# mattsaccount364/FractalShark

Measured on AMD Instinct MI355X. Metric: Mpix/s (iteration buffer), View #5 3840x2160 HDRx32 LAv2, higher is better.
Workload: dtype f32+i32exp; 1 GPU; view5_3840x2160_hdrx32_lav2_full; parity=cpu, kernel_variant=tuned, frames=warm: frames of one view back to back

## Files before the change

fractalshark_amd/_capi.py:

```python
import ctypes as C
import os

from . import _build

vp = C.c_void_p
u32 = C.c_uint32
u64 = C.c_uint64
i32 = C.c_int32


class RealHdr32(C.Structure):
    _fields_ = [("m", C.c_float), ("e", C.c_int32)]


class CplxHdr32(C.Structure):
    _fields_ = [("re", C.c_float), ("im", C.c_float), ("e", C.c_int32)]


class AtHdr32(C.Structure):
    _fields_ = [("StepLength", u32), ("ThresholdC", RealHdr32), ("SqrEscapeRadius", RealHdr32),
                ("RefC", CplxHdr32), ("ZCoeff", CplxHdr32), ("CCoeff", CplxHdr32), ("InvZCoeff", CplxHdr32),
                ("CCoeffSqrInvZCoeff", CplxHdr32), ("CCoeffInvZCoeff", CplxHdr32),
                ("CCoeffNormSqr", RealHdr32), ("RefCNormSqr", RealHdr32), ("factor", RealHdr32)]

# ... 55 lines not shown
    fn.argtypes = argtypes
    return fn


def render_lib():
    global _render
    if _render is not None:
        return _render
    path = os.environ.get("FSMI355_LIB") or _build.LIB_RENDER
    if os.environ.get("FSMI355_LIB"):
        import sys
        print("fractalshark_amd: FSMI355_LIB overrides the in-tree library: %s" % path, file=sys.stderr)
    if not os.path.exists(path):
        raise RuntimeError("libfsmi355.so is missing (%s): run `python -c 'import __graft_entry__ as g; g.build()'`"
                           % path)
    lib = C.CDLL(path)
    _decl(lib, "fs_create", vp, [C.c_int])
    _decl(lib, "fs_destroy", None, [vp])
    _decl(lib, "fs_test_device_is_working", u32, [])
    _decl(lib, "fs_device_count", C.c_int, [])
    _decl(lib, "fs_host_fallback_bytes", u64, [vp])
    _decl(lib, "fs_idle_device_bytes", u64, [vp])
    _decl(lib, "fs_release_idle_device_memory", u64, [C.c_int])
    _decl(lib, "fs_set_compressed_orbit_mode", u32, [vp, C.c_int])
    _decl(lib, "fs_orbit_device_bytes", u64, [vp])
    _decl(lib, "fs_error_string", C.c_char_p, [u32])
    _decl(lib, "fs_init_memory", u32, [vp, u32, u32, u32, u32, vp, u32, u32, u64, C.c_int])
    _decl(lib, "fs_set_row_bands", u32, [vp, u32, u32, u32])
    _decl(lib, "fs_local_rows", u32, [vp])
    _decl(lib, "fs_set_external_iter_buffer", u32, [vp, vp, u64])
    _decl(lib, "fs_device_iter_buffer", vp, [vp])
    _decl(lib, "fs_rounded_width", u32, [vp])
    _decl(lib, "fs_upload_orbit", u32, [vp, u64, C.c_int, u32, vp, u64, u64, u64])
    _decl(lib, "fs_upload_orbit_compressed", u32, [vp, u64, C.c_int, u32, vp, u64, u64, u64, vp, vp])
    _decl(lib, "fs_upload_la", u32, [vp, u64, C.c_int, u32, vp, u32, vp, u32, C.c_int, C.c_int, vp])
    _decl(lib, "fs_upload_bla", u32, [vp, C.c_int, vp, vp, i32, i32])
    _decl(lib, "fs_render_lav2", u32, [vp, C.c_int, C.c_int, C.c_int, vp, u64])
    _decl(lib, "fs_feature_eval", u32, [vp, C.c_int, u32, C.c_int, vp, u64, vp, vp, u64])
    _decl(lib, "fs_feature_eval_direct", u32, [vp, C.c_int, u32, C.c_int, vp, u64, vp, vp, u64])
    _decl(lib, "fs_set_feature_slice", u32, [vp, u32])
    _decl(lib, "fs_autozoom_pick", u32, [vp, C.c_int, u64, vp, C.POINTER(AutozoomResult)])
    _decl(lib, "fs_set_autozoom_gather_cap", u32, [vp, u32])
    _decl(lib, "fs_render_exact", u32, [vp, u32, u32, u32, vp, vp, u32, C.c_int, u64])
    _decl(lib, "fs_exact_stable_mask", u32, [vp, u32, u32, vp, vp, u32, u64, vp])
    _decl(lib, "fs_set_exact_slice", u32, [vp, u32, C.c_int])
    _decl(lib, "fs_read_exact_stats", u32, [vp, vp])
    _decl(lib, "fs_exact_sample_counts", u32, [vp, u32, u32, vp, vp, u32, u32, C.c_int, u64, vp])
    _decl(lib, "fs_render_exact_wide", u32, [vp, u32, u32, u32, vp, vp, u32, C.c_int, u64])
    _decl(lib, "fs_exact_wide_state", u32, [vp, u32, u32, vp, vp, u32, u32, vp, vp])
    _decl(lib, "fs_render_bla", u32, [vp, C.c_int, vp, u64])
    _decl(lib, "fs_render_direct", u32, [vp, C.c_int, vp, u64])
    _decl(lib, "fs_upload_orbit_scaled", u32, [vp, C.c_int, u32, vp, vp, u64, u64])
    _decl(lib, "fs_render_scaled", u32, [vp, C.c_int, vp, u64])
    _decl(lib, "fs_build_bla", u32, [vp, C.c_int, vp])
    _decl(lib, "fs_bla_num_levels", i32, [vp])
    _decl(lib, "fs_bla_lm2", i32, [vp])
    _decl(lib, "fs_bla_level_size", u64, [vp, i32])
    _decl(lib, "fs_read_bla_level", u32, [vp, i32, vp, u64])
    _decl(lib, "fs_render_direct_lp", u32, [vp, C.c_int, vp, u64, C.c_int])
    _decl(lib, "fs_clear", u32, [vp])
    _decl(lib, "fs_render_current", u32, [vp, u64, vp, vp, vp, C.c_int])
    _decl(lib, "fs_sync_compute", u32, [vp])
    _decl(lib, "fs_compute_stream", vp, [vp])
    _decl(lib, "fs_sync_display", u32, [vp])
    _decl(lib, "fs_query_compute", u32, [vp])
    _decl(lib, "fs_enqueue_done_callback", u32, [vp, DONE_CB, vp])
    _decl(lib, "fs_get_width", u32, [vp])
    _decl(lib, "fs_get_height", u32, [vp])
    _decl(lib, "fs_last_kernel_ms", C.c_float, [vp])
    _decl(lib, "fs_set_kernel_variant", u32, [vp, C.c_int])
    _decl(lib, "fs_kernel_ms_history", u32, [vp, vp, u32])
    _decl(lib, "fs_kernel_ms_split_history", u32, [vp, vp, vp, u32])
    _decl(lib, "fs_forget_tile_costs", u32, [vp])
    _decl(lib, "fs_last_frame_tile_ordered", C.c_int, [vp])
    _decl(lib, "fs_last_frame_sampled_tile_order", C.c_int, [vp])
    _decl(lib, "fs_read_tile_costs", u32, [vp, vp, u64, vp])
    _decl(lib, "fs_read_tile_order", u32, [vp, vp, u64])
    _decl(lib, "fs_seq_cursor_probe", u32, [vp, C.c_int, u64, u32, vp])
    _decl(lib, "fs_enable_step_count", u32, [vp, C.c_int])
    _decl(lib, "fs_read_step_count", u32, [vp, vp])
    _decl(lib, "fs_time_render_current", u32, [vp, u64, u32, vp])
    _decl(lib, "fs_read_stats_raw", u32, [vp, vp, u64])
    _decl(lib, "fs_test_block_threshold", u32, [vp, vp, vp, vp, vp, u32])
    _decl(lib, "fs_build_la", u32, [vp, C.c_int, vp, C.c_int])
    _decl(lib, "fs_build_la_mt", u32, [vp, C.c_int, vp, C.c_int, C.c_int])
    _decl(lib, "fs_la_counts", u32, [vp, vp, vp, vp, vp])
    _decl(lib, "fs_read_la", u32, [vp, vp, u32, vp, u32, vp])
    _decl(lib, "fs_group_create", vp, [vp, C.c_int, C.c_int])
    _decl(lib, "fs_group_destroy", None, [vp])
    _decl(lib, "fs_group_size", C.c_int, [vp])
    _decl(lib, "fs_group_transport", C.c_int, [vp])
    _decl(lib, "fs_group_renderer", vp, [vp, C.c_int])
    _decl(lib, "fs_group_init_memory", u32, [vp, u32, u32, u32, u32, vp, u32, u32, u64])
    _decl(lib, "fs_group_upload_orbit", u32, [vp, u64, C.c_int, u32, vp, u64, u64, u64])
    _decl(lib, "fs_group_upload_orbit_compressed", u32, [vp, u64, C.c_int, u32, vp, u64, u64, u64, vp, vp])
    _decl(lib, "fs_group_upload_la", u32, [vp, u64, C.c_int, u32, vp, u32, vp, u32, C.c_int, C.c_int, vp])
    _decl(lib, "fs_group_upload_bla", u32, [vp, C.c_int, vp, vp, i32, i32])
    _decl(lib, "fs_group_upload_orbit_scaled", u32, [vp, C.c_int, u32, vp, vp, u64, u64])
    _decl(lib, "fs_group_render_lav2", u32, [vp, C.c_int, C.c_int, C.c_int, vp, u64])
    _decl(lib, "fs_group_render_bla", u32, [vp, C.c_int, vp, u64])
    _decl(lib, "fs_group_render_scaled", u32, [vp, C.c_int, vp, u64])
    _decl(lib, "fs_group_render_direct", u32, [vp, C.c_int, vp, u64])
    _decl(lib, "fs_group_clear", u32, [vp])
    _decl(lib, "fs_group_render_current", u32, [vp, u64, vp, vp])
    _decl(lib, "fs_group_render_current_colors", u32, [vp, u64, vp, vp, vp, C.c_int])
    _decl(lib, "fs_group_sync_display", u32, [vp])
    _decl(lib, "fs_display_stream", vp, [vp])
    _decl(lib, "fs_colorize_frame", u32, [vp, vp, u64, vp, vp, vp])
    _decl(lib, "fs_color_buffer_elements", u64, [vp])
    _decl(lib, "fs_group_sync", u32, [vp])
    _decl(lib, "fs_group_wait_current", u32, [vp, u32])
    _decl(lib, "fs_group_gather_ms", C.c_float, [vp])
    _decl(lib, "fs_group_plan", None, [u32, u32, u32, u32, vp, vp, vp])
    _decl(lib, "fs_group_set_host_path", u32, [vp, C.c_int])
    _decl(lib, "fs_group_host_path", C.c_int, [vp])
    _decl(lib, "fs_copy_bands_to_host", u32, [vp, vp, vp, vp])
    _decl(lib, "fs_host_register", u32, [vp, u64])
    _decl(lib, "fs_host_unregister", u32, [vp])
    _render = lib
    return lib


RENDER_SYMBOLS = [
    "fs_create", "fs_destroy", "fs_test_device_is_working", "fs_device_count", "fs_error_string", "fs_init_memory", "fs_set_row_bands",
    "fs_local_rows", "fs_set_external_iter_buffer", "fs_device_iter_buffer", "fs_rounded_width", "fs_upload_orbit", "fs_upload_orbit_compressed",
    "fs_upload_la", "fs_upload_bla", "fs_render_lav2", "fs_feature_eval", "fs_feature_eval_direct", "fs_set_feature_slice",
    "fs_autozoom_pick", "fs_set_autozoom_gather_cap",
    "fs_render_exact", "fs_exact_stable_mask", "fs_set_exact_slice", "fs_read_exact_stats",
    "fs_exact_sample_counts", "fs_render_exact_wide", "fs_exact_wide_state",
    "fs_render_bla", "fs_render_direct", "fs_upload_orbit_scaled",
    "fs_render_scaled", "fs_build_bla", "fs_bla_num_levels", "fs_bla_lm2", "fs_bla_level_size", "fs_read_bla_level",
    "fs_render_direct_lp", "fs_clear",
    "fs_render_current", "fs_sync_compute", "fs_compute_stream", "fs_sync_display", "fs_query_compute", "fs_enqueue_done_callback",
    "fs_host_fallback_bytes", "fs_idle_device_bytes", "fs_release_idle_device_memory", "fs_set_compressed_orbit_mode", "fs_orbit_device_bytes", "fs_get_width", "fs_get_height", "fs_last_kernel_ms", "fs_set_kernel_variant", "fs_kernel_ms_history", "fs_kernel_ms_split_history", "fs_forget_tile_costs", "fs_last_frame_tile_ordered", "fs_last_frame_sampled_tile_order", "fs_read_tile_costs", "fs_read_tile_order", "fs_seq_cursor_probe", "fs_enable_step_count", "fs_read_step_count",
    "fs_time_render_current", "fs_read_stats_raw", "fs_test_block_threshold", "fs_build_la", "fs_build_la_mt", "fs_la_counts", "fs_read_la",
    "fs_group_create", "fs_group_destroy", "fs_group_size", "fs_group_transport", "fs_group_renderer", "fs_group_init_memory",
    "fs_group_upload_orbit", "fs_group_upload_orbit_compressed", "fs_group_upload_la", "fs_group_upload_bla",
    "fs_group_upload_orbit_scaled", "fs_group_render_lav2", "fs_group_render_bla", "fs_group_render_scaled",
    "fs_group_render_direct", "fs_group_clear", "fs_group_render_current", "fs_group_render_current_colors", "fs_group_sync_display", "fs_display_stream", "fs_colorize_frame",
    "fs_color_buffer_elements", "fs_group_sync", "fs_group_wait_current", "fs_group_gather_ms",
    "fs_group_plan", "fs_group_set_host_path", "fs_group_host_path", "fs_copy_bands_to_host", "fs_host_register", "fs_host_unregister",
]


def inputs_lib():
    global _inputs
    if _inputs is not None:
        return _inputs
    path = _build.LIB_INPUTS
    if not os.path.exists(path):
        raise RuntimeError("libfsinputs.so is missing (%s): run __graft_entry__.build()" % path)
    lib = C.CDLL(path)
    _decl(lib, "fsh_view_create", vp, [C.c_char_p] * 4 + [u32, u32])
    _decl(lib, "fsh_view_destroy", None, [vp])
    _decl(lib, "fsh_view_autozoom_next", vp, [vp, C.c_double, C.c_double, u32, u32, u32])
    _decl(lib, "fsh_view_save_im", C.c_int, [vp, u64, C.c_char_p, C.c_int])
    _decl(lib, "fsh_view_load_im", vp, [C.c_char_p, u32, u32, C.POINTER(u64), C.POINTER(C.c_int), C.POINTER(C.c_int)])
    _decl(lib, "fsh_view_precision_bits", u64, [vp])
    _decl(lib, "fsh_view_exact_axes", C.c_int, [vp, u32, u32, u32, C.c_int, u32, vp, vp])
    _decl(lib, "fsh_view_bbox_str", C.c_int, [vp, C.c_int, C.c_char_p, C.c_size_t])
    _decl(lib, "fsh_view_coords_direct_f64", None, [vp, u32, u32, vp])
    _decl(lib, "fsh_view_coords_direct_hdr32", None, [vp, u32, u32, vp])
    _decl(lib, "fsh_view_coords_direct_hdr64", None, [vp, u32, u32, vp])
    _decl(lib, "fsh_orbit_create", vp, [vp, C.c_int, u64, C.c_int])
    _decl(lib, "fsh_orbit_create_ex", vp, [vp, C.c_int, u64, C.c_int, C.c_int])
    _decl(lib, "fsh_orbit_is_compressed", C.c_int, [vp])
    _decl(lib, "fsh_orbit_compressed_count", u64, [vp])
    _decl(lib, "fsh_orbit_compressed_data_hdr32", vp, [vp])
    _decl(lib, "fsh_orbit_low_hdr32", None, [vp, vp])
    _decl(lib, "fsh_orbit_compressed_data_hdr64", vp, [vp])
    _decl(lib, "fsh_orbit_low_hdr64", None, [vp, vp])
    _decl(lib, "fsh_la_default_params", None, [C.POINTER(C.c_int32)])
    _decl(lib, "fsh_mpz_raw_write", C.c_size_t, [C.c_char_p, C.c_int, C.c_char_p, C.c_size_t])
    _decl(lib, "fsh_mpz_raw_read", C.c_size_t, [C.c_char_p, C.c_size_t, C.c_char_p, C.c_size_t])
    _decl(lib, "fsh_orbit_save_im", C.c_int, [vp, u64, C.c_int, C.c_char_p, C.c_int])
    _decl(lib, "fsh_orbit_load_im", vp, [C.c_char_p, C.POINTER(u64)])
    _decl(lib, "fsh_orbit_is64", C.c_int, [vp])
    _decl(lib, "fsh_orbit_destroy", None, [vp])
    _decl(lib, "fsh_feature_begin", vp, [vp, vp, u32, u32, u32, u64])
    _decl(lib, "fsh_feature_begin_direct", vp, [vp, C.c_int, u32, u32, u32, u64])
    _decl(lib, "fsh_feature_begin_direct_at", vp, [vp, C.c_int, u32, u32, u32, u64])
    _decl(lib, "fsh_feature_direct_grid", C.c_int, [vp, C.c_int, u32, u32, vp, vp])
    _decl(lib, "fsh_feature_destroy", None, [vp])
    _decl(lib, "fsh_feature_is64", C.c_int, [vp])
    _decl(lib, "fsh_feature_candidates", u64, [vp])
    _decl(lib, "fsh_feature_next_batch", u64, [vp, vp, u64, C.POINTER(C.c_int), vp, C.POINTER(u64)])
    _decl(lib, "fsh_feature_consume", None, [vp, vp, u64])
    _decl(lib, "fsh_feature_found", u64, [vp])
    _decl(lib, "fsh_feature_result", C.c_int, [vp, u64, C.c_char_p, C.c_char_p, C.c_char_p, C.c_size_t, C.POINTER(u64),
                                                vp, C.POINTER(u32)])
    _decl(lib, "fsh_orbit_count", u64, [vp])
    _decl(lib, "fsh_orbit_scale_entries", u64, [vp, vp, vp, u64])
    _decl(lib, "fsh_orbit_period", u64, [vp])
    _decl(lib, "fsh_orbit_data_hdr32", vp, [vp])
    _decl(lib, "fsh_orbit_data_hdr64", vp, [vp])
    _decl(lib, "fsh_orbit_max_radius_hdr32", None, [vp, vp])
    _decl(lib, "fsh_orbit_max_radius_hdr64", None, [vp, vp])
    _decl(lib, "fsh_orbit_data_hdr32_bad", vp, [vp])
    _decl(lib, "fsh_orbit_data_f32_bad", vp, [vp])
    _decl(lib, "fsh_orbit_bad_count", u64, [vp])
    _decl(lib, "fsh_view_coords_direct_lp", None, [vp, u32, u32, C.c_int, vp])
    _decl(lib, "fsh_view_coords_perturb_hdr32", None, [vp, vp, u32, u32, vp])
    _decl(lib, "fsh_view_coords_perturb_hdr64", None, [vp, vp, u32, u32, vp])
    _decl(lib, "fsh_df32_op", None, [C.c_int, vp, vp, vp])
    _decl(lib, "fsh_hr2_reduce", None, [vp])
    _decl(lib, "fsh_hr2_add", None, [vp, vp, C.c_int, vp])
    _decl(lib, "fsh_hc2_reduce", None, [vp])
    _decl(lib, "fsh_convert_orbit_hdr64_to_2x32", None, [vp, u64, vp])
    _decl(lib, "fsh_convert_la_hdr64_to_2x32", None, [vp, u64, vp])
    _decl(lib, "fsh_convert_at_hdr64_to_2x32", None, [vp, vp])
    _decl(lib, "fsh_view_coords_perturb_2x32", None, [vp, vp, u32, u32, vp])
    _decl(lib, "fsh_la_create_hdr32", vp, [vp, C.c_int])
    _decl(lib, "fsh_la_create", vp, [vp, C.c_int])
    _decl(lib, "fsh_la_create_ex", vp, [vp, C.c_int, C.c_int])
    _decl(lib, "fsh_la_is64", C.c_int, [vp])
    _decl(lib, "fsh_la_destroy", None, [vp])
    _decl(lib, "fsh_la_count", u32, [vp])
    _decl(lib, "fsh_la_data", vp, [vp])
# ... 55 lines not shown
```

fractalshark_amd/csrc/kernels.h:

```cpp
#pragma once

#include <hip/hip_runtime.h>
#include <stdint.h>

#include "../../include/fs_layout.h"
#include "exact_math.hpp"
#include "exact_wide_math.hpp"
#include "hdr_math.hpp"

enum { FS_MODE_FULL = 0, FS_MODE_PO = 1, FS_MODE_LAO = 2 };
enum { FS_PARITY_LITERAL = 0, FS_PARITY_GPUSTAGE = 1 };
enum { FS_VARIANT_TUNED = 0, FS_VARIANT_LITERAL = 1, FS_VARIANT_TUNED_NOSCALE = 2, FS_VARIANT_BASE_MASK = 0xff };
enum { FS_VARIANT_FLAG_LDS_ORBIT = 0x100, FS_VARIANT_FLAG_REFILL = 0x200, FS_VARIANT_FLAG_WIDE = 0x400,
       FS_VARIANT_FLAG_NATURAL_ORDER = 0x800, FS_VARIANT_FLAG_BLA_POOL = 0x1000 };

struct FsFrame {
    uint32_t width;
    uint32_t height;
    uint32_t rounded_width;
    uint32_t local_rows;
    uint32_t band_first;
    uint32_t band_rows;
    uint32_t band_stride;
    uint32_t iter_u64;
    uint32_t wide;
};

struct FsZ64 {
    double re;
    double im;
    int32_t e;
    int32_t pad_;
    double w;
};
template <class F> struct FsDev;
template <> struct FsDev<float> {
    using Z = float4;
    using Orbit = fs_orbit_hdr32;
    using Real = fs_real_hdr32;
    using Cplx = fs_cplx_hdr32;
    using LA = fs_la_hdr32_u32;
    using AT = fs_at_hdr32_u32;
    using BLA = fs_bla_hdr32;
};
template <> struct FsDev<double> {
    using Z = FsZ64;
    using Orbit = fs_orbit_hdr64;
    using Real = fs_real_hdr64;
    using Cplx = fs_cplx_hdr64;
    using LA = fs_la_hdr64_u32;
    using AT = fs_at_hdr64_u32;
    using BLA = fs_bla_hdr64;
};

template <class F> struct FsFeatRec;
template <> struct FsFeatRec<float> {
    using In = fs_feature_in_hdr32;
    using Out = fs_feature_out_hdr32;
};
template <> struct FsFeatRec<double> {
    using In = fs_feature_in_hdr64;
    using Out = fs_feature_out_hdr64;
};
template <class F> struct FsFeatLane {
    fs::hcplx<F> z, dz, dzdc, zcoeff, dc, c;
    fs::hreal<F> sqr_r, sqr_scale;
    uint64_t step, cap, period;
    uint32_t ref, phase;
};
template <class F> struct FsFeatDirectLane {
    fs::hcplx<F> z, dzdc, zcoeff, c;
    uint64_t step, cap, period;
    uint32_t phase, pad_;
};

template <class F> struct FsCoordsT {
    fs::hreal<F> dx, dy, centerX, centerY;
};
using FsCoords32 = FsCoordsT<float>;

struct FsAtRes {
    double re, im;
    int32_t e;
    uint32_t i;
};
template <class F> struct FsLav2ArgsT {
    uint32_t *out;
    const typename FsDev<F>::Z *zref;
    const float4 *zq;
    const float4 *zs;
    const float2 *zs2;
    const float4 *zqb;
    const typename FsDev<F>::LA *las;
    const fs_la_stage_u32 *stages;
    uint64_t *stats;
    FsFrame frame;
    FsCoordsT<F> coords;
    typename FsDev<F>::AT at;
    uint32_t orbit_count;
    uint32_t period;
    uint32_t stage_count;
    uint32_t n_iterations;
    uint32_t n_iterations_hi;
    int la_valid;
    int use_at;
    int parity;
    const void *wp;
    uint32_t n_wp;
    typename FsDev<F>::Real cxLow, cyLow;
    const uint32_t *tile_order;
    uint32_t *tile_cost;
    uint32_t tiles_x;
    const uint32_t *pixel_order;
    uint32_t *pixel_cost;
    struct FsAtRes *at_res;
    uint32_t *at_cost;
    uint32_t orbit_count_hi, period_hi, at_step_hi, la_u64;
};
using FsLav2Args32 = FsLav2ArgsT<float>;
template <class F> struct FsLaU64;
template <> struct FsLaU64<float> {
    using T = fs_la_hdr32_u64;
};
template <> struct FsLaU64<double> {
    using T = fs_la_hdr64_u64;
};

struct FsBlaRec {
    float Axm, Aym, Bxm, Bym;
    int32_t Axe, Aye, Bxe, Bye;
    float Zre, Zim;
    int32_t Ze;
    uint32_t l;
};
static_assert(sizeof(FsBlaRec) == 48, "device-native BLA record");
constexpr int kBlaMaxLevels = 40;

template <class F> struct FsBlaArgsT {
    uint32_t *out;
    const typename FsDev<F>::Z *zref;
    const float4 *zq;
    const float4 *zs;
    const float2 *zs2;
    const float4 *zqb;
    const typename FsDev<F>::BLA *const *levels;
    uint64_t *stats;
    uint32_t *queue;
    const uint32_t *tile_order;
    uint32_t *probe_out;
    uint32_t probe_pitch;
    FsFrame frame;
    FsCoordsT<F> coords;
    uint32_t orbit_count;
    uint32_t n_iterations;
    uint32_t n_iterations_hi;
    int32_t lm2;
    const FsBlaRec *nrec;
    const int4 *nlad;
    const long long *nkmax;
    uint32_t level_off[kBlaMaxLevels];
    const float4 *zb;
    const int4 *hq;
    const int4 *hlad;
    const FsBlaRec *hrec;
};
using FsBlaArgs32 = FsBlaArgsT<float>;

struct FsBlaArgsF64 {
    uint32_t *out;
    const fs_orbit_f64 *orbit;
    const fs_bla_f64 *const *levels;
    uint64_t *stats;
    FsFrame frame;
    double dx, dy, centerX, centerY;
    uint32_t orbit_count;
    uint32_t n_iterations;
    uint32_t n_iterations_hi;
    int32_t lm2;
};

template <class F> struct FsDirectHdrArgsT {
    uint32_t *out;
    fs::hreal<F> *cx_row;
    uint64_t *stats;
    FsFrame frame;
    fs::hreal<F> dy;
    fs::hreal<F> maxY;
    uint32_t n_iterations;
    uint32_t n_iterations_hi;
};

struct FsLav2Args2x32 {
    uint32_t *out;
    const fs_orbit_2x32 *orbit;
    const fs_la_2x32_u32 *las;
    const fs_la_stage_u32 *stages;
    uint64_t *stats;
    FsFrame frame;
    fs_real_2x32 coords[4];
    fs_at_2x32_u32 at;
    uint32_t orbit_count;
    uint32_t stage_count;
    uint32_t n_iterations;
    uint32_t n_iterations_hi;
    int la_valid;
    int use_at;
    const fs_orbit_2x32_rc *wp;
    uint32_t n_wp;
    fs_real_2x32 cxLow, cyLow;
    const uint32_t *pixel_order;
    uint32_t *pixel_cost;
    const uint32_t *tile_order;
    uint32_t tiles_x;
};

struct FsLav2ArgsPlain {
    uint32_t *out;
    const void *orbit;
    const void *las;
    const fs_la_stage_u32 *stages;
    uint64_t *stats;
    FsFrame frame;
    alignas(8) uint8_t at[sizeof(fs_at_f64_u32)];
    alignas(8) uint8_t coords[4 * sizeof(double)];
    uint32_t orbit_count;
    uint32_t stage_count;
    uint32_t n_iterations;
    uint32_t n_iterations_hi;
    int la_valid;
    int use_at;
    const void *wp;
    uint32_t n_wp;
    alignas(8) uint8_t c_low[2][8];
};

struct FsScaledArgs32 {
    uint32_t *out;
    const fs_orbit_hdr32_bad *orbit_t;
    const fs_orbit_f32_bad *orbit_f;
    uint64_t *stats;
    FsFrame frame;
    FsCoordsT<float> coords;
    uint32_t orbit_count;
    uint32_t n_iterations;
    uint32_t n_iterations_hi;
    float w2threshold;
};

struct FsScaledArgsF64 {
    uint32_t *out;
    const fs_orbit_f64_bad *orbit_t;
    const fs_orbit_f32_bad *orbit_f;
    uint64_t *stats;
    FsFrame frame;
    double dx, dy, centerX, centerY;
    uint32_t orbit_count;
    uint32_t n_iterations;
    uint32_t n_iterations_hi;
    float w2threshold;
};

struct FsDirectLpArgs {
    uint32_t *out;
    uint64_t *stats;
    FsFrame frame;
    float c32[16];
    double c64[16];
    uint32_t n_iterations;
    uint32_t n_iterations_hi;
};

struct FsDirectArgs64 {
    uint32_t *out;
    double *cx_row;
    uint64_t *stats;
    FsFrame frame;
    double dy;
    double maxY;
    uint32_t n_iterations;
    uint32_t n_iterations_hi;
};

void fsk_prepare_orbit_hdr32(const fs_orbit_hdr32 *in, float4 *out, uint64_t n, hipStream_t s);
void fsk_decompress_orbit_plain(int type_tag, const void *wp, uint64_t n_wp, uint64_t n_uncompressed, const void *cxLow,
                                const void *cyLow, void *out, hipStream_t s);
void fsk_decompress_orbit_hdr32(const fs_orbit_hdr32_rc *wp, uint64_t n_wp, uint64_t n_uncompressed, fs_real_hdr32 cxLow,
                                fs_real_hdr32 cyLow, float4 *out, hipStream_t s);
void fsk_decompress_orbit_hdr64(const fs_orbit_hdr64_rc *wp, uint64_t n_wp, uint64_t n_uncompressed, fs_real_hdr64 cxLow,
                                fs_real_hdr64 cyLow, FsZ64 *out, hipStream_t s);
void fsk_prepare_orbit_hdr64(const fs_orbit_hdr64 *in, FsZ64 *out, uint64_t n, hipStream_t s);
template <class F>
void fsk_feature_init(const void *in, FsFeatLane<F> *st, void *out, uint64_t n, int find, fs::hreal<F> R, uint64_t max_iters,
                      uint64_t count, hipStream_t s);
template <class F>
void fsk_feature_step(const typename FsDev<F>::Z *zref, uint32_t count, FsFeatLane<F> *st, void *out, uint64_t n, int find,
                      int iter_u64, uint32_t slice, uint32_t *unfinished, hipStream_t s);
template <class F>
void fsk_feature_direct_init(const void *in, FsFeatDirectLane<F> *st, void *out, uint64_t n, int find, fs::hreal<F> R,
                             uint64_t max_iters, hipStream_t s);
template <class F>
void fsk_feature_direct_step(FsFeatDirectLane<F> *st, void *out, uint64_t n, int find, int iter_u64, fs::hreal<F> R,
                             uint32_t slice, uint32_t *unfinished, hipStream_t s);
void fsk_make_quiet_orbit(const float4 *zref, float4 *zq, float2 *zs2, float4 *zqb, uint64_t n, hipStream_t s);
void fsk_tile_order(const uint32_t *probe, uint32_t probe_pitch, uint32_t tiles_x, uint32_t tiles_y, uint32_t threshold,
                    uint32_t *order, uint32_t n_slots, hipStream_t s);
uint32_t fsk_tile_order_work_words(uint32_t n_tiles);
void fsk_tile_order_by_cost(const uint32_t *cost, uint32_t n_tiles, uint32_t *tmp, uint32_t *order, uint32_t n_slots,
                            hipStream_t s);
uint32_t fsk_lav2_hdr32_slots(const FsFrame &f);
void fsk_lav2_hdr32(const FsLav2Args32 &A, int mode, bool stats, int variant, hipStream_t s);
void fsk_lav2_hdr64(const FsLav2ArgsT<double> &A, int mode, bool stats, hipStream_t s);
void fsk_at_pass64(const FsLav2ArgsT<double> &A, hipStream_t s);
void fsk_lav2_wide(const FsLav2Args32 *A32, const FsLav2ArgsT<double> *A64, int mode, bool stats, hipStream_t s);
void fsk_lav2_seq(const FsLav2Args32 *A32, const FsLav2ArgsT<double> *A64, int mode, bool stats, hipStream_t s);
void fsk_seq_cursor_probe(bool is64, bool wide_pos, const void *wp, uint32_t n_wp, const void *cx, const void *cy,
                          uint64_t start, uint32_t n, void *out, hipStream_t s);
void fsk_lav2_2x32(const FsLav2Args2x32 &A, int mode, bool stats, hipStream_t s);
void fsk_lav2_plain(const FsLav2ArgsPlain &A, int kind, int mode, bool stats, hipStream_t s);
bool fsk_direct_lp(const FsDirectLpArgs &A, int kind, int iteration_precision, bool stats, hipStream_t s);
void fsk_scaled_hdr32(const FsScaledArgs32 &A, bool stats, int variant, hipStream_t s);
void fsk_scaled_bounds(fs_orbit_f32_bad *of, uint64_t n, hipStream_t s);
void fsk_scaled_f64(const FsScaledArgsF64 &A, bool stats, int variant, hipStream_t s);
void fsk_bla_build_hdr32(const float4 *zref, void *const *levels, const uint64_t *epl, int n_levels, fs_real_hdr32 bla_size,
                         hipStream_t s);
void fsk_bla_build_hdr64(const FsZ64 *zref, void *const *levels, const uint64_t *epl, int n_levels, fs_real_hdr64 bla_size,
                         hipStream_t s);
void fsk_bla_make_native(const fs_bla_hdr32 *const *levels, const uint32_t *level_off, const uint64_t *epl, int n_levels,
                         const float4 *zref, uint32_t orbit_count, FsBlaRec *rec, int4 *lad, uint32_t *bad, int32_t lm2, long long *kmax, uint32_t n_kmax, hipStream_t s);
void fsk_perturb_scalar_hdr32(const FsBlaArgs32 &A, bool use_bla, bool stats, int variant, hipStream_t s);
uint64_t fsk_bla_heap_positions(const uint64_t *epl, int n_levels);
void fsk_bla_make_heap(const FsBlaRec *rec, const int4 *lad, const long long *kmax, uint32_t n_kmax, const uint32_t *level_off,
                       const uint64_t *epl, int n_levels, int32_t lm2, const float4 *zref, uint32_t orbit_count, FsBlaRec *hrec,
                       int4 *hlad, int4 *hq, float4 *zb, hipStream_t s);
void fsk_bla_hdr32_fast(const FsBlaArgs32 &A, bool pool, hipStream_t s);
struct FsTileSampleArgs {
    FsFrame frame;
    FsCoordsT<double> coords;
    fs::hreal<double> ThresholdC, SqrEscapeRadius;
    fs::hcplx<double> RefC, CCoeff;
    uint32_t StepLength;
    uint32_t n_iterations;
    uint32_t tiles_x, tiles_y;
    uint32_t n_slots;
    uint32_t *cost;
};
void fsk_at_tile_sample64(const FsTileSampleArgs &A, hipStream_t s);
void fsk_tile_order_finish(uint32_t *order, uint32_t n_slots, uint32_t n_tiles, hipStream_t s);
size_t fsk_pixel_order_temp_bytes(uint32_t n);
hipError_t fsk_pixel_order_build(const uint32_t *counts, uint32_t n, uint32_t *work, uint32_t *order, void *temp, size_t temp_bytes,
                                 hipStream_t s);
void fsk_lav2_lit32(const FsLav2Args32 &A, int mode, bool stats, dim3 g, dim3 b, hipStream_t s);
void fsk_lav2_hdr64_fast(const FsLav2ArgsT<double> &A, int mode, bool stats, hipStream_t s);
void fsk_perturb_scalar_hdr64(const FsBlaArgsT<double> &A, bool use_bla, bool stats, int variant, hipStream_t s);
void fsk_perturb_bla_f64(const FsBlaArgsF64 &A, bool use_bla, bool stats, hipStream_t s);
void fsk_direct_hdr32(const FsDirectHdrArgsT<float> &A, fs::hreal<float> minX, fs::hreal<float> dx, bool stats, hipStream_t s);
void fsk_direct_hdr64(const FsDirectHdrArgsT<double> &A, fs::hreal<double> minX, fs::hreal<double> dx, bool stats,
                      hipStream_t s);
void fsk_direct_f64(const FsDirectArgs64 &A, double minX, double dx, bool stats, hipStream_t s);
void fsk_antialias(const void *iters, int iter_u64, uint32_t rounded_width, fs_color16 *colors, const fs_color16 *pal,
                   uint32_t pal_iters, uint32_t aux_depth, uint32_t aa, uint32_t color_w, uint32_t color_h,
                   uint64_t n_iterations, hipStream_t s);
void fsk_reduce(const void *iters, int iter_u64, uint32_t rounded_width, uint32_t width, uint32_t rows,
                fs_reduction *out, hipStream_t s);
struct FsAzStats {
    uint64_t max_iter, sum, n_ge;
    uint64_t num_at_limit, first_index, num_at_max;
    uint64_t candidates, accepted, run_reject, hist[9];
    uint64_t best_key;
    uint64_t gathered;
    double sums[3];
};
struct FsAzTipRec {
    uint32_t x, y;
    uint64_t iter;
    uint32_t high, pad_;
};
struct FsAzFrame {
    const void *iters;
    uint32_t iter_u64, pitch, W, H;
    uint64_t n_iterations;
};
void fsk_az_stats(const FsAzFrame &F, uint32_t x0, uint32_t y0, uint32_t w, uint32_t h, FsAzStats *st, hipStream_t s);
void fsk_az_max(const FsAzFrame &F, FsAzStats *st, hipStream_t s);
void fsk_az_default(const FsAzFrame &F, uint32_t x0, uint32_t y0, uint32_t w, uint32_t h, double width_over_2,
                    double height_over_2, double max_distance, FsAzStats *st, double *slab, hipStream_t s);
void fsk_az_tip_score(const FsAzFrame &F, double max_dist, FsAzStats *st, hipStream_t s);
// ... 3 lines not shown
struct FsExactArgs {
    const uint32_t *cx, *cy;
    uint32_t W, H, rounded_width;
    uint32_t iter_u64;
    void *iters;
    uint64_t cap;
    fsx::Params P;
    const uint32_t *src_xy;
    const uint64_t *src_n;
    const uint32_t *src_pix;
    uint32_t *dst_xy;
    uint64_t *dst_n;
    uint32_t *dst_pix;
    uint32_t stride;
    uint32_t n_src;
    uint32_t first;
    uint32_t compact;
    uint32_t slice;
    uint32_t *dst_count;
    unsigned long long *stats;
};
bool fsk_exact_slice(const FsExactArgs &A, uint32_t limbs, hipStream_t s);
void fsk_exact_mask(const void *centre, const void *shifted, int iter_u64, uint8_t *mask, uint32_t W, uint32_t H, uint32_t pitch,
                    int first, hipStream_t s);

struct FsExactWideArgs {
    const uint32_t *cx, *cy;
    uint32_t nx, ny;
    uint32_t W;
    uint32_t out_pitch;
    uint32_t out_u64;
    void *out;
    uint64_t cap;
    uint32_t limbs;
    fsx::Params P;
    const uint32_t *src_xy;
    const uint64_t *src_n;
    const uint32_t *src_id;
    uint32_t *dst_xy;
    uint64_t *dst_n;
    uint32_t *dst_id;
    uint32_t stride;
    uint32_t first;
    uint32_t state_only;
    uint32_t slice;
    uint32_t *dst_count;
    unsigned long long *stats;
};
bool fsk_exact_wide_slice(const FsExactWideArgs &A, uint32_t n_src, hipStream_t s);

void fsk_gather_rows(const void *in, void *out, const uint32_t *index, uint32_t row_bytes, uint32_t rows, hipStream_t s);

template <class F> void fsk_la_src_orbit(const void *zref, uint32_t n, void *chebv, hipStream_t s);
template <class F> void fsk_la_src_stage(const void *P, uint32_t n, void *chebv, void *mm, uint32_t *steps, hipStream_t s);
void fsk_scan_u32(const uint32_t *in, uint32_t *out, uint32_t n, hipStream_t s);
template <class F> void fsk_la_first(bool stage0, const void *chebv, const void *mm, uint32_t limit, uint32_t *out, hipStream_t s);
template <class F>
void fsk_la_first_from(const void *chebv, const uint32_t *bases, uint32_t n_queries, uint32_t limit, uint32_t *out, hipStream_t s);
template <class F>
void fsk_la_records_list(const void *zref, const uint32_t *seg, uint32_t n, void *out, void *tail_out, uint32_t max_ref,
                         hipStream_t s);
template <class F>
void fsk_la_next(bool stage0, const void *chebv, const void *mm, const uint32_t *pos, uint32_t limit, uint32_t period,
                 uint32_t *next, uint32_t *reach, uint32_t x_start, hipStream_t s);
void fsk_la_reach(const uint32_t *jin, uint32_t *jout, uint32_t *reach, uint32_t nstates, hipStream_t s);
void fsk_la_mail(const uint32_t *src, uint32_t n, uint32_t *mail, uint32_t seq, hipStream_t s);
void fsk_la_reach_all(const uint32_t *next, uint32_t *bufB, uint32_t *bufC, uint32_t *reach, uint32_t nstates, uint32_t rounds,
                      hipStream_t s);
template <class F>
void fsk_la_records(bool stage0, const void *zref, const void *P, const uint32_t *pos, const uint32_t *next,
                    const uint32_t *reach, const uint32_t *rank, uint32_t limit, uint32_t rank_offset, void *out, void *tail_out,
                    uint32_t max_ref, hipStream_t s);
template <class F>
void fsk_la_stage_prologue(const void *P, const void *chebv, const void *mm, const uint32_t *steps, uint32_t *pos, uint32_t count,
                           uint32_t *out, hipStream_t s);
template <class F>
void fsk_la_one_record(bool stage0, const void *zref, const void *P, uint32_t e, uint32_t step_length, void *out, hipStream_t s);
template <class F> void fsk_la_tail(const void *zref, uint32_t max_ref, void *out, uint32_t *zcoeff_zero, hipStream_t s);
template <class F>
void fsk_la_at(const void *las, const uint32_t *stage_la_index, uint32_t stage_count, const void *radius,
               int use_small_exponents, void *at_out, uint32_t *use_at, hipStream_t s);
void fsk_la_pack(bool is64, const void *in, void *out, uint32_t n, hipStream_t s);
void fsk_test_block_threshold(const int *bw, const int *eshm, const int *sdc, int *t_out, uint32_t n, hipStream_t s);
```

fractalshark_amd/csrc/kernels.hip:

```cpp
#include <hip/hip_runtime.h>
#include <stdint.h>

#include <type_traits>

#include "../../include/fs_layout.h"
#include "hdr_math.hpp"
#include "at_math.hpp"
#include "kernels.h"
#include <cstdlib>
#include "kernel_common.hpp"
#include "lav2_common.hpp"
#include "scaled_runs.hpp"

using namespace fs;


__global__ void k_prepare_orbit_hdr32(const fs_orbit_hdr32 *__restrict__ in, float4 *__restrict__ out, uint64_t n)
{
    const uint64_t i = (uint64_t)blockIdx.x * blockDim.x + threadIdx.x;
    if (i >= n)
        return;
    const fs_orbit_hdr32 e = in[i];
    const hcplx32 c = hc_from_hr(hreal32{e.mx, e.ex}, hreal32{e.my, e.ey});
    out[i] = make_float4(c.re, c.im, __int_as_float(c.e), ldexpf(1.0f, 8 - 2 * (c.e < -1000 ? -1000 : c.e)));
}

__device__ __forceinline__ float scaled_bound(const float4 v)
{
    const int e = __float_as_int(v.z);
    const float hi = fs_max_abs(v.x, v.y);
    const float lo = fs_min_abs(v.x, v.y);
    const float zmax = __builtin_amdgcn_ldexpf(hi, e < -200 ? -200 : (e > 100 ? 100 : e));
    const bool usable = zmax >= 0x1p-40f && zmax < 5.6f && lo >= hi * 0x1p-40f;
    return usable ? zmax * 0x1p-2f : -0.0f;
}


__device__ __forceinline__ float scaled_block_bound(const float4 *__restrict__ zref, uint64_t j, uint64_t n)
{
    if (j >= n)
        return -0.0f;
    float best = 0x1p60f, grow = 1.0f;
    bool ok = true;
    for (uint32_t k = 0; k < 4; k++) {
        const float4 v = zref[j + k < n ? j + k : n - 1];
        const int e = __float_as_int(v.z);
        const float m = __builtin_amdgcn_ldexpf(fs_max_abs(v.x, v.y),
                                               e < -200 ? -200 : (e > 100 ? 100 : e));
        ok = ok && m < 5.6f;
        grow *= (4.0f * m + 3.8f) * (1.0f + 0x1p-10f);
        const float bk = j + k + 1 < n ? scaled_bound(zref[j + k + 1]) : -0.0f;
        ok = ok && __float_as_int(bk) != (int)0x80000000;
        best = __builtin_fminf(best, bk / grow);
    }
    return ok ? best * (1.0f - 0x1p-10f) : -0.0f;
}

__global__ void k_make_quiet_orbit(const float4 *__restrict__ zref, float4 *__restrict__ zq, float2 *__restrict__ zs2,
                                   float4 *__restrict__ zqb, uint64_t n)
{
    const uint64_t i = (uint64_t)blockIdx.x * blockDim.x + threadIdx.x;
    if (i >= n)
        return;
    const float4 v = zref[i];
    const int e = __float_as_int(v.z);
    zq[i] = make_float4(v.x, v.y, __int_as_float(e <= 2 ? ~e + 116 : (1 << 24)), 0.0f);
    const float b0 = scaled_bound(v);
    zq[n + i] = make_float4(__builtin_amdgcn_ldexpf(v.x, e + 1), __builtin_amdgcn_ldexpf(v.y, e + 1), b0,
                            scaled_block_bound(zref, i, n));
    zs2[i] = make_float2(__builtin_amdgcn_ldexpf(v.x, e + 1), __builtin_amdgcn_ldexpf(v.y, e + 1));
    zqb[i] = make_float4(scaled_block_bound(zref, i + 3, n), scaled_block_bound(zref, i + 7, n),
                         scaled_block_bound(zref, i + 11, n), scaled_block_bound(zref, i + 15, n));
}

namespace {

template <class F> struct FsWaypoints;
template <> struct FsWaypoints<float> {
    using Rec = fs_orbit_hdr32_rc;
};
template <> struct FsWaypoints<double> {
    using Rec = fs_orbit_hdr64_rc;
};

template <class F, class PosT = uint32_t> struct SeqOrbit {
    const typename FsWaypoints<F>::Rec *__restrict__ wp;
    uint32_t n_wp;
    hreal<F> cx, cy;
    PosT idx;
    uint32_t next;
    PosT next_index;
    hreal<F> zx, zy;

    __device__ __forceinline__ PosT index_of(uint32_t k) const
    {
        return (PosT)(wp[k].index_and_rebase & 0x7FFFFFFFFFFFFFFFull);
    }
    __device__ __forceinline__ void load(uint32_t k)
    {
        zx = hreal<F>{wp[k].mx, wp[k].ex};
        zy = hreal<F>{wp[k].my, wp[k].ey};
    }
    __device__ __forceinline__ void step()
    {
        idx++;
        if (idx == next_index) {
            load(next);
            next++;
            next_index = next < n_wp ? index_of(next) : ~(PosT)0;
        } else {
            const hreal<F> zx_old = zx;
            zx = hr_add(hr_sub(hr_mul(zx, zx), hr_mul(zy, zy)), cx);
            hr_reduce(zx);
            zy = hr_add(hr_mul(hr_mul(hreal<F>{F(1), 1}, zx_old), zy), cy);
            hr_reduce(zy);
        }
    }
    __device__ __forceinline__ void seek(PosT i)
    {
        uint32_t lo = 0, hi = n_wp;
        while (hi - lo > 1u) {
            const uint32_t mid = (lo + hi) >> 1;
            if (index_of(mid) <= i)
                lo = mid;
            else
                hi = mid;
        }
        load(lo);
        idx = index_of(lo);
        next = lo + 1u;
        next_index = next < n_wp ? index_of(next) : ~(PosT)0;
        while (idx < i)
            step();
    }
    __device__ __forceinline__ hcplx<F> value() const { return hc_from_hr(zx, zy); }
};

template <class F, class PosT>
__global__ void k_seq_cursor_probe(const void *wp, uint32_t n_wp, hreal<F> cx, hreal<F> cy, uint64_t start, uint32_t n,
                                   hcplx<F> *out)
{
    if (threadIdx.x != 0 || blockIdx.x != 0)
        return;
    SeqOrbit<F, PosT> seq;
    seq.wp = (const typename FsWaypoints<F>::Rec *)wp;
    seq.n_wp = n_wp;
    seq.cx = cx, seq.cy = cy;
    seq.seek((PosT)start);
    for (uint32_t k = 0; k < n; k++) {
        out[k] = seq.value();
        seq.step();
    }
}

}
// ... 405 lines not shown
        while (iter < n_iterations) {
            if (kBla) {
                const fs_bla_f64 *b;
                while ((b = bla_lookup_f64(A, RefIteration, DeltaNormSquared)) != nullptr) {
                    const uint32_t l = (uint32_t)b->l;
                    if (RefIteration + l >= count)
                        break;
                    if (iter + l >= n_iterations)
                        break;
                    iter += l;
                    if (kStats)
                        c_la++;
                    {
                        const double Ax = b->Ax, Ay = b->Ay, Bx = b->Bx, By = b->By;
                        const double nx = Ax * DeltaSubNX - Ay * DeltaSubNY + Bx * DeltaSub0X - By * DeltaSub0Y;
                        const double ny = Ax * DeltaSubNY + Ay * DeltaSubNX + Bx * DeltaSub0Y + By * DeltaSub0X;
                        DeltaSubNX = nx;
                        DeltaSubNY = ny;
                    }
                    RefIteration += l;
                    const fs_orbit_f64 Z = orbit[RefIteration];
                    const double tempZX = Z.x + DeltaSubNX;
                    const double tempZY = Z.y + DeltaSubNY;
                    const double normSquared = tempZX * tempZX + tempZY * tempZY;
                    DeltaNormSquared = DeltaSubNX * DeltaSubNX + DeltaSubNY * DeltaSubNY;
                    if (normSquared > 256.0)
                        break;
                    if (normSquared < DeltaNormSquared || RefIteration >= count - 1) {
                        DeltaSubNX = tempZX;
                        DeltaSubNY = tempZY;
                        DeltaNormSquared = normSquared;
                        RefIteration = 0;
                    }
                }
                if (iter >= n_iterations)
                    break;
            }
            const double OX = DeltaSubNX, OY = DeltaSubNY;
            const fs_orbit_f64 Z = orbit[RefIteration];
            const double TermB1 = OX * (Z.x * 2 + OX);
            const double TermB2 = OY * (Z.y * 2 + OY);
            DeltaSubNX = TermB1 - TermB2;
            DeltaSubNX += DeltaSub0X;
            const double Term3 = Z.y * 2 + OY;
            const double Term4 = Z.x * 2 + OX;
            DeltaSubNY = OX * Term3 + OY * Term4;
            DeltaSubNY += DeltaSub0Y;
            if (kStats)
                c_pt++;
            ++RefIteration;
            if (RefIteration >= count)
                break;
            const fs_orbit_f64 Z2 = orbit[RefIteration];
            const double tempZX = Z2.x + DeltaSubNX;
            const double tempZY = Z2.y + DeltaSubNY;
            const double nT1 = tempZX * tempZX;
            const double nT2 = tempZY * tempZY;
            const double normSquared = nT1 + nT2;
            DeltaNormSquared = DeltaSubNX * DeltaSubNX + DeltaSubNY * DeltaSubNY;
            if (normSquared > 256.0)
                break;
            if (normSquared < DeltaNormSquared || RefIteration >= count - 1) {
                DeltaSubNX = tempZX;
                DeltaSubNY = tempZY;
                DeltaNormSquared = normSquared;
                RefIteration = 0;
            }
            ++iter;
        }
        store_iter(A.out, A.frame, L, X, iter);
    }
    if (kStats)
        add_stats(A.stats, 0, c_la, c_pt, c_px);
}

static dim3 frame_grid(const FsFrame &f) { return dim3((f.width + 63) / 64, (f.local_rows + 3) / 4, 1); }
static dim3 tile_grid(const FsFrame &f) { return dim3((f.width + 31) / 32, (f.local_rows + 7) / 8, 1); }

void fsk_prepare_orbit_hdr32(const fs_orbit_hdr32 *in, float4 *out, uint64_t n, hipStream_t s)
{
    hipLaunchKernelGGL(k_prepare_orbit_hdr32, dim3((unsigned)((n + 255) / 256)), dim3(256), 0, s, in, out, n);
}

void fsk_make_quiet_orbit(const float4 *zref, float4 *zq, float2 *zs2, float4 *zqb, uint64_t n, hipStream_t s)
{
    hipLaunchKernelGGL(k_make_quiet_orbit, dim3((unsigned)((n + 255) / 256)), dim3(256), 0, s, zref, zq, zs2, zqb, n);
}

__global__ void k_decompress_orbit_hdr64(const fs_orbit_hdr64_rc *__restrict__ wp, uint64_t n_wp, uint64_t n_uncompressed,
                                         fs_real_hdr64 cxLow, fs_real_hdr64 cyLow, FsZ64 *__restrict__ out)
{
    const uint64_t k = (uint64_t)blockIdx.x * blockDim.x + threadIdx.x;
    if (k >= n_wp)
        return;
    const uint64_t kIndexMask = 0x7FFFFFFFFFFFFFFFull;
    const uint64_t i0 = wp[k].index_and_rebase & kIndexMask;
    const uint64_t i1 = k + 1 < n_wp ? (wp[k + 1].index_and_rebase & kIndexMask) : n_uncompressed;
    hreal64 zx{wp[k].mx, wp[k].ex}, zy{wp[k].my, wp[k].ey};
    const hreal64 cx = ldr(cxLow), cy = ldr(cyLow);
    const hreal64 Two{1.0, 1};
    for (uint64_t i = i0; i < i1 && i < n_uncompressed; i++) {
        const hcplx64 c = hc_from_hr(zx, zy);
        FsZ64 z;
        z.re = c.re;
        z.im = c.im;
        z.e = c.e;
        z.pad_ = 0;
        z.w = ldexp(1.0, 8 - 2 * (c.e < -500 ? -500 : c.e));
        out[i] = z;
        const hreal64 zx_old = zx;
        zx = hr_add(hr_sub(hr_mul(zx, zx), hr_mul(zy, zy)), cx);
        hr_reduce(zx);
        zy = hr_add(hr_mul(hr_mul(Two, zx_old), zy), cy);
        hr_reduce(zy);
    }
}

void fsk_decompress_orbit_hdr64(const fs_orbit_hdr64_rc *wp, uint64_t n_wp, uint64_t n_uncompressed, fs_real_hdr64 cxLow,
                                fs_real_hdr64 cyLow, FsZ64 *out, hipStream_t s)
{
    hipLaunchKernelGGL(k_decompress_orbit_hdr64, dim3((unsigned)((n_wp + 63) / 64)), dim3(64), 0, s, wp, n_wp,
                       n_uncompressed, cxLow, cyLow, out);
}

void fsk_decompress_orbit_hdr32(const fs_orbit_hdr32_rc *wp, uint64_t n_wp, uint64_t n_uncompressed, fs_real_hdr32 cxLow,
                                fs_real_hdr32 cyLow, float4 *out, hipStream_t s)
{
    hipLaunchKernelGGL(k_decompress_orbit_hdr32, dim3((unsigned)((n_wp + 63) / 64)), dim3(64), 0, s, wp, n_wp,
                       n_uncompressed, cxLow, cyLow, out);
}

void fsk_prepare_orbit_hdr64(const fs_orbit_hdr64 *in, FsZ64 *out, uint64_t n, hipStream_t s)
{
    hipLaunchKernelGGL(k_prepare_orbit_hdr64, dim3((unsigned)((n + 255) / 256)), dim3(256), 0, s, in, out, n);
}

__global__ void __launch_bounds__(256) k_at_pass64(FsLav2ArgsT<double> A)
{
    using F = double;
    uint32_t X, L;
    if (A.pixel_order)
        ordered_pixel(A.frame, A.pixel_order, X, L);
    else
        tile_pixel(X, L);
    const bool in_buffer = X < A.frame.width && L < A.frame.local_rows;
    const uint32_t Y = in_buffer ? global_row(A.frame, L) : 0xFFFFFFFFu;
    if (!(in_buffer && Y < A.frame.height))
        return;
    hreal<F> deltaReal, deltaImaginary;
    pixel_delta<F>(A.coords, X, Y, deltaReal, deltaImaginary);
    const hcplx<F> DeltaSub0 = hc_from_hr(deltaReal, deltaImaginary);
    FsAtRes out{0.0, 0.0, 0, 0xFFFFFFFFu};
    uint32_t own = 0;
    if (A.la_valid && A.use_at && hr_cmp_pos(hc_cheb(DeltaSub0), ldr(A.at.ThresholdC)) <= 0) {
        const uint32_t ATMaxIt = A.n_iterations / A.at.StepLength;
        hcplx<F> c = hc_add(hc_mul(DeltaSub0, ldc(A.at.CCoeff)), ldc(A.at.RefC));
        hc_reduce(c);
        hcplx<F> z;
        uint32_t i, i_exec = 0, i_own = 0;
        at_perform<F, uint32_t>(c, ldr(A.at.SqrEscapeRadius), ATMaxIt, z, i, &i_exec, &i_own);
        hcplx<F> dz = hc_mul(z, ldc(A.at.InvZCoeff));
        hc_reduce(dz);
        out = FsAtRes{dz.re, dz.im, dz.e, i};
        own = i_own;
    }
    const size_t idx = (size_t)L * A.frame.rounded_width + X;
    A.at_res[idx] = out;
    if (A.at_cost)
        A.at_cost[idx] = own;
// ... 187 lines not shown
```

fractalshark_amd/csrc/kernels_lav2_hdr32.hip:

```cpp
#include <hip/hip_runtime.h>
#include <stdint.h>

#include <type_traits>

#include "../../include/fs_layout.h"
#include "hdr_math.hpp"
#include "at_math.hpp"
#include "kernels.h"
#include <cstdlib>
#include "kernel_common.hpp"
#include "lav2_common.hpp"
#include "scaled_runs.hpp"

using namespace fs;

__global__ void k_test_block_threshold(const int *__restrict__ bw, const int *__restrict__ eshm, const int *__restrict__ sdc,
                                       int *__restrict__ t_out, uint32_t n)
{
    const uint32_t i = blockIdx.x;
    if (i >= n)
        return;
    const int b = __builtin_amdgcn_readfirstlane(bw[i]), e = __builtin_amdgcn_readfirstlane(eshm[i]),
              d = __builtin_amdgcn_readfirstlane(sdc[i]);
    int t;
    asm volatile("s_mov_b32 s67, %[b]\n\t" FS_BT_T("s67") : [t] "=&s"(t) : [b] "s"(b), [eshm] "s"(e), [sdc] "s"(d) : "s67", "scc");
    if (threadIdx.x == 0)
        t_out[i] = t;
}

void fsk_test_block_threshold(const int *bw, const int *eshm, const int *sdc, int *t_out, uint32_t n, hipStream_t s)
{
    hipLaunchKernelGGL(k_test_block_threshold, dim3(n), dim3(64), 0, s, bw, eshm, sdc, t_out, n);
}

template <int Mode, bool kStats, bool kScaled, bool kLds = false, bool kGpuStage = false>
__global__ void __launch_bounds__(256) __attribute__((amdgpu_waves_per_eu(7, 8))) k_lav2_hdr32_fast(FsLav2Args32 A)
{
    __shared__ float4 s_zs_lds[kLds ? 4 * 2 * 64 : 1];
    __shared__ uint32_t s_it0[256];
    __shared__ float4 s_dcp[256];
    __shared__ float s_dzp[2 * 256];
    uint32_t tile_x, tile_y;
    const uint32_t wave_in_block = (uint32_t)__builtin_amdgcn_readfirstlane((int)(threadIdx.x >> 6));
    if (A.tile_order) {
        const uint32_t w = (blockIdx.y * gridDim.x + blockIdx.x) * (blockDim.x >> 6) + wave_in_block;
        const uint32_t tile = (uint32_t)__builtin_amdgcn_readfirstlane((int)A.tile_order[w]);
        tile_y = tile != 0xFFFFFFFFu ? tile / A.tiles_x : 0u;
        tile_x = tile != 0xFFFFFFFFu ? tile - tile_y * A.tiles_x : 0xFFFFFFFu;
    } else {
        tile_x = blockIdx.x * (blockDim.x >> 6) + wave_in_block;
        tile_y = blockIdx.y;
    }
    uint32_t X, L;
    uint32_t lds_lane16 = 0;
    {
        uint32_t lane;
        asm volatile("v_mbcnt_lo_u32_b32 %0, -1, 0\n\tv_mbcnt_hi_u32_b32 %0, -1, %0" : "=v"(lane));
        X = tile_x * 8u + (lane & 7u);
        L = tile_y * 8u + (lane >> 3);
        if constexpr (kLds)
            asm volatile("v_lshlrev_b32_e32 %0, 4, %1" : "=v"(lds_lane16) : "v"(lane));
    }
    uint32_t lane_cost = 0;
#ifdef FS_TRACE_WAVES
    const uint64_t trace_t0 = wall_clock64();
#endif
    uint64_t c_at = 0, c_la = 0, c_pt = 0, c_px = 0;
    uint64_t c_careful = 0, c_scaled = 0, c_runs = 0;
    uint32_t c_why[4] = {0, 0, 0, 0};
    uint32_t c_nz[4] = {0, 0, 0, 0};
    bool was_skip = false;
    uint32_t c_wentry = 0, c_wstart = 0, c_wshort = 0;
    uint32_t c_blk_violation = 0;
    uint32_t c_pass = 0, c_generic = 0;
    uint32_t c_blk_free = 0, c_blk_tested = 0;
    uint32_t c_lane_steps = 0, c_lane_runs = 0;
    uint32_t c_nd_steps = 0, c_nd_fail = 0, c_nd_replayed = 0, c_nd_mismatch = 0;
#ifdef FS_PROFILE_CYCLES
    uint64_t cyc_loop = 0, cyc_run = 0, cyc_body = 0, cyc_t0 = 0, cyc_t1 = 0, cyc_t2 = 0;
    uint64_t cyc_asm = 0, cyc_tested = 0, cyc_hot = 0, cyc_t3 = 0, cyc_t4 = 0, cyc_t5 = 0, wall_loop = 0, wall_t0 = 0;
#define FS_CYC(stmt) do { if (kStats) { stmt; } } while (0)
#else
#define FS_CYC(stmt) do { } while (0)
#endif
    const uint32_t Y = global_row(A.frame, L);
    const bool live = X < A.frame.width && L < A.frame.local_rows && Y < A.frame.height;
    if (live) {
        c_px = 1;
        const uint32_t n_iterations = A.n_iterations;
        hreal32 deltaReal, deltaImaginary;
        pixel_delta<float>(A.coords, X, Y, deltaReal, deltaImaginary);
        const hcplx32 DeltaSub0 = hc_from_hr(deltaReal, deltaImaginary);
        hcplx32 DeltaSubN = hc_from_native<float>(0.0f, 0.0f);
        uint32_t iterations = 0;
        uint32_t la_cost = 0;

        if (Mode != FS_MODE_PO) {
            if (A.la_valid && A.use_at && hr_cmp_pos(hc_cheb(DeltaSub0), ldr(A.at.ThresholdC)) <= 0) {
                const uint32_t ATMaxIt = n_iterations / A.at.StepLength;
                hcplx32 c = hc_add(hc_mul(DeltaSub0, ldc(A.at.CCoeff)), ldc(A.at.RefC));
                hc_reduce(c);
                hcplx32 z;
                uint32_t i;
                at_perform<float>(c, ldr(A.at.SqrEscapeRadius), ATMaxIt, z, i);
                hcplx32 dz = hc_mul(z, ldc(A.at.InvZCoeff));
                hc_reduce(dz);
                DeltaSubN = dz;
                iterations = i * A.at.StepLength;
                la_cost = i;
                if (kStats)
                    c_at = i;
            }
        }

        uint32_t RefIteration = 0;
        const uint32_t MaxRefIteration = A.orbit_count - 1;
        if (iterations != 0 && !(RefIteration < MaxRefIteration) && A.period != 0)
            RefIteration = RefIteration % A.period;

        if (Mode != FS_MODE_PO) {
            uint32_t CurrentLAStage = A.la_valid ? A.stage_count : 0;
            const hreal32 dcCheb = hc_cheb(DeltaSub0);
            while (CurrentLAStage > 0) {
                CurrentLAStage--;
                const uint32_t LAIndex = A.stages[CurrentLAStage].LAIndex;
                {
                    const int cmp = hr_cmp_pos(dcCheb, ldr(A.las[LAIndex].LAThresholdC));
                    const bool invalid = kGpuStage ? (cmp >= 0) : (cmp < 0);
                    if (invalid)
                        continue;
                }
                const uint32_t MacroItCount = A.stages[CurrentLAStage].MacroItCount;
                uint32_t j = RefIteration;
                hcplx32 RefJ = hc_zero<float>();
                if (iterations < n_iterations)
                    RefJ = ldc(A.las[LAIndex + j].Ref);
                while (iterations < n_iterations) {
                    const fs_la_hdr32_u32 *LAj = &A.las[LAIndex + j];
                    const uint32_t l = LAj->StepLength;
                    bool unusable = true;
                    hcplx32 newDz = hc_zero<float>();
                    if (iterations + l <= n_iterations) {
                        newDz = hc_mul(DeltaSubN, hc_add(hc_mul2(RefJ), DeltaSubN));
                        hc_reduce(newDz);
                        unusable = hr_cmp_pos(hc_cheb(newDz), ldr(LAj->LAThreshold)) >= 0;
                    }
                    if (unusable) {
                        RefIteration = LAj->NextStageLAIndex;
                        break;
                    }
                    iterations += l;
                    la_cost += 8u;
                    if (kStats)
                        c_la++;
                    if (__builtin_amdgcn_ballot_w64(fs::clamp_exp(newDz.e + LAj->ZCoeff.e) - fs::clamp_exp(DeltaSub0.e + LAj->CCoeff.e) >=
                                                    fs::kExpDiffIgnored) == __builtin_amdgcn_ballot_w64(true))
                        DeltaSubN = hc_mul(newDz, ldc(LAj->ZCoeff));
                    else
                        DeltaSubN = hc_add(hc_mul(newDz, ldc(LAj->ZCoeff)), hc_mul(DeltaSub0, ldc(LAj->CCoeff)));
                    const hcplx32 RefN = ldc(LAj[1].Ref);
// ... 292 lines not shown
                                    for (uint32_t e8 = 0; e8 < steps_here; e8 += 8u) {
                                        const float4 ua = cb[e8], ub = cb[e8 + 1], uc = cb[e8 + 2], ud = cb[e8 + 3];
                                        const float4 ue = cb[e8 + 4], uf = cb[e8 + 5], ug = cb[e8 + 6], uh = cb[e8 + 7];
                                        f2 t1, u1;
                                        uint64_t v1 = 0;
                                        FS_SCALED_STEP(w0, z0, t1, u1, a, v1, false, (void)0, ua.x, ua.y, ua.z);
                                        FS_SCALED_STEP(t1, u1, w2, z2, b, v1, true, (void)0, ub.x, ub.y, ub.z);
                                        if (v1 != 0ull) {
                                            FS_TRIP_FAILED(a, t1, ua.z, w0)
                                            run_over = true;
                                            break;
                                        }
                                        c += 2;
                                        f2 t3, u3;
                                        uint64_t v2 = 0;
                                        FS_SCALED_STEP(w2, z2, t3, u3, c_, v2, false, (void)0, uc.x, uc.y, uc.z);
                                        FS_SCALED_STEP(t3, u3, w0, z0, d, v2, true, (void)0, ud.x, ud.y, ud.z);
                                        if (v2 != 0ull) {
                                            FS_TRIP_FAILED(c_, t3, uc.z, w2)
                                            run_over = true;
                                            break;
                                        }
                                        c += 2;
                                        f2 t5, u5;
                                        uint64_t v3 = 0;
                                        FS_SCALED_STEP(w0, z0, t5, u5, e, v3, false, (void)0, ue.x, ue.y, ue.z);
                                        FS_SCALED_STEP(t5, u5, w2, z2, f, v3, true, (void)0, uf.x, uf.y, uf.z);
                                        if (v3 != 0ull) {
                                            FS_TRIP_FAILED(e, t5, ue.z, w0)
                                            run_over = true;
                                            break;
                                        }
                                        c += 2;
                                        f2 t7, u7;
                                        uint64_t v4 = 0;
                                        FS_SCALED_STEP(w2, z2, t7, u7, g, v4, false, (void)0, ug.x, ug.y, ug.z);
                                        FS_SCALED_STEP(t7, u7, w0, z0, h, v4, true, (void)0, uh.x, uh.y, uh.z);
                                        if (v4 != 0ull) {
                                            FS_TRIP_FAILED(g, t7, ug.z, w2)
                                            run_over = true;
                                            break;
                                        }
                                        c += 2;
                                    }
                                    if (run_over)
                                        break;
                                    chunk++;
                                    if (c >= run_len) {
                                        wO = w0, failed = false;
                                        run_over = true;
                                    }
                                }
                                asm volatile("s_waitcnt vmcnt(0)" ::: "memory");
#undef FS_GLDS_CHUNK
                            } else {
                            typedef float f4 __attribute__((ext_vector_type(4)));
                            const float4 *zpu = zs + ref_u + 1;
#if defined(FS_VERIFY_BLOCK_BOUND) || defined(FS_VERIFY_FLOOR)
                            const int imdc = __float_as_int(fs_max_abs(dcs.x, dcs.y));
#endif
                            const int Esh_cap = wave_upper_bound_i32(Esh);
                            int nd_form = 0;
                            if (!fl_per_trip) {
                                if (nd_skip != 0u) {
                                    nd_skip--;
                                } else {
                                    const float f_run = __builtin_fmaxf(FS_FL_FLOOR, __builtin_amdgcn_ldexpf(fs_max_abs(dcs.x, dcs.y), 26));
                                    const bool nd_ok = f_run < __builtin_inff() && mn0 * __builtin_amdgcn_ldexpf(1.0f, -kScaleShift) >= f_run;
                                    if (__builtin_amdgcn_ballot_w64(!nd_ok) == 0ull)
                                        nd_form = 1;
                                    else
                                        nd_skip = kNdBackoffEntry;
                                }
                            }
                            float mxS = mx0 * __builtin_amdgcn_ldexpf(1.0f, -kScaleShift);
                            int pwi = __builtin_amdgcn_readfirstlane(__float_as_int(e0.w));
                            f2 zS = {__int_as_float(__builtin_amdgcn_readfirstlane(__float_as_int(e0.x))),
                                     __int_as_float(__builtin_amdgcn_readfirstlane(__float_as_int(e0.y)))};
                            f2 wv = w0;
                            uint32_t cs = 0;
                            const uint32_t rl = (uint32_t)__builtin_amdgcn_readfirstlane((int)run_len);
                            const uint32_t lim8 = (rl << 4) - 0x80u;
                            const float4 *const zpb = zpu;
                            for (;;) {
#ifdef FS_VERIFY_BLOCK_BOUND
                                const long long bt_d = (long long)pwi - (long long)Esh_cap;
                                const int bt_thr = sdc_bits > pwi ? -1 : (bt_d > 0x46800000ll ? 0x46800000 : (int)bt_d);
                                const bool bt_pass = __builtin_amdgcn_ballot_w64(__float_as_int(mxS) > bt_thr) == 0ull;
                                if (kStats && bt_pass)
                                    c_blk_free++;
#else
                                {
                                    f2 r1, r2, r3 = wv, ts_, ta_;
                                    uint64_t xacc_ = 0;
                                    float tn_, tl_;
                                    uint64_t msk_;
                                    int st, ebo, pf_, pg_, ph_, bt_t_;
                                    const uint32_t c_in = cs;
                                    uint32_t off = cs << 4;
                                    FS_CYC(cyc_t3 = __builtin_readcyclecounter());
#ifndef FS_VERIFY_FLOOR
                                    if (!fl_per_trip) {
                                        {
                                            int nd_sel = __builtin_amdgcn_readfirstlane(nd_form);
                                            if (kStats && nd_form != 0) {
                                                const f2 wv_s = wv, zS_s = zS;
                                                const float mxS_s = mxS;
                                                const int pwi_s = pwi;
                                                const uint32_t off_s = off;
                                                FS_FAST_LOOP_FDU(FS_PF_NONE);
                                                const int st_n = __builtin_amdgcn_readfirstlane(st);
                                                if (st_n != 5 && st_n != 3) {
                                                    const f2 wv_n = wv, zS_n = zS;
                                                    const float mxS_n = mxS;
                                                    const int pwi_n = pwi;
                                                    const uint32_t off_n = off;
                                                    wv = wv_s, zS = zS_s, mxS = mxS_s, pwi = pwi_s, off = off_s;
                                                    nd_sel = 0;
                                                    FS_FAST_LOOP_FDU(FS_PF_NONE);
                                                    const bool lane_diff = __float_as_int(wv.x) != __float_as_int(wv_n.x) ||
                                                                           __float_as_int(wv.y) != __float_as_int(wv_n.y) ||
                                                                           __float_as_int(mxS) != __float_as_int(mxS_n);
                                                    const bool wave_diff =
                                                        __builtin_amdgcn_readfirstlane(st) != st_n ||
                                                        __builtin_amdgcn_readfirstlane((int)off) != __builtin_amdgcn_readfirstlane((int)off_n) ||
                                                        __builtin_amdgcn_readfirstlane(pwi) != __builtin_amdgcn_readfirstlane(pwi_n) ||
                                                        __builtin_amdgcn_readfirstlane(__float_as_int(zS.x)) !=
                                                            __builtin_amdgcn_readfirstlane(__float_as_int(zS_n.x)) ||
                                                        __builtin_amdgcn_readfirstlane(__float_as_int(zS.y)) !=
                                                            __builtin_amdgcn_readfirstlane(__float_as_int(zS_n.y));
                                                    c_nd_replayed++;
                                                    if (wave_diff || __builtin_amdgcn_ballot_w64(lane_diff) != 0ull)
                                                        c_nd_mismatch++;
                                                    wv = wv_n, zS = zS_n, mxS = mxS_n, pwi = pwi_n, off = off_n;
                                                    st = st_n;
                                                }
                                            } else {
                                                FS_FAST_LOOP_FDU(FS_PF_NONE);
                                            }
                                        }
                                        ebo = 0;
                                    } else
#endif
                                    {
#if !(defined(FS_VERIFY_BLOCK_BOUND) || defined(FS_VERIFY_FLOOR))
                                        const int imdc = __float_as_int(fs_max_abs(dcs.x, dcs.y));
#endif
                                        FS_FAST_LOOP_FL(FS_PF_NONE);
                                    }
#ifdef FS_VERIFY_FLOOR
                                    if (kStats && xacc_ != 0ull)
                                        c_blk_violation++;
#endif
                                    FS_CYC(cyc_asm += __builtin_readcyclecounter() - cyc_t3);
                                    st = __builtin_amdgcn_readfirstlane(st);
                                    zS = (f2){__int_as_float(__builtin_amdgcn_readfirstlane(__float_as_int(zS.x))),
                                              __int_as_float(__builtin_amdgcn_readfirstlane(__float_as_int(zS.y)))};
                                    if (st == 3) {
                                        fl_redo = true;
                                        break;
                                    }
                                    if (st == 5) {
                                        fl_redo = nd_redo = true;
                                        if (kStats)
                                            c_nd_fail++;
                                        break;
                                    }
                                    cs = (uint32_t)__builtin_amdgcn_readfirstlane((int)off) >> 4;
                                    if (kStats && nd_form != 0)
                                        c_nd_steps += cs - c_in;
                                    pwi = __builtin_amdgcn_readfirstlane(pwi);
                                    if (kStats)
                                        c_blk_free += (cs - c_in) >> 2;
                                    if (st != 0) {
                                        const float ebf = __int_as_float(__builtin_amdgcn_readfirstlane(ebo));
                                        c = cs;
                                        if (st == 1) {
                                            FS_TRIP_FAILED_NB(a, r1, ebf, wv)
                                        } else {
                                            FS_TRIP_FAILED_NB(a, r3, ebf, r2)
                                        }
                                        break;
                                    }
                                }
#endif
                                if (cs + 4u > rl) {
                                    c = cs, wO = wv, failed = false;
                                    break;
                                }
                                if (__builtin_amdgcn_ballot_w64(!(mxS < FS_FL_HIGH)) != 0ull) {
                                    c = cs, wO = wv, failed = false;
                                    break;
                                }
                                if (kStats)
                                    c_blk_tested++;
                                FS_CYC(cyc_t4 = __builtin_readcyclecounter());
                                typedef float f16 __attribute__((ext_vector_type(16)));
                                f16 U;
                                asm volatile("s_load_dwordx16 %0, %1, 0x0" : "=s"(U) : "s"(zpb + cs));
                                f2 tp_, tq_;
                                FS_STEP_ARITH(wv, zS, tp_, a)
                                asm volatile("s_waitcnt lgkmcnt(0)" : "+s"(U), "+v"(tp_));
                                const f4 ua = U.s0123, ub = U.s4567, uc = U.s89ab, ud = U.scdef;
                                const f2 up_ = {ua.x, ua.y}, uq_ = {uc.x, uc.y};
                                uint64_t vp_ = 0, vq_ = 0;
                                c = cs;
                                FS_STEP_BOUND(tp_, a, vp_, ua.z)
                                FS_STEP_FLOOR_FIRST(tp_, vp_)
                                FS_STEP_ARITH(tp_, up_, w2, b)
                                FS_STEP_BOUND(w2, b, vp_, ub.z)
                                FS_STEP_FLOOR(w2, vp_)
#ifdef FS_VERIFY_BLOCK_BOUND
                                if (kStats && bt_pass &&
                                    (__builtin_amdgcn_ballot_w64(__float_as_int(mx_a) + Esh > __float_as_int(ua.z)) |
                                     __builtin_amdgcn_ballot_w64(__float_as_int(mx_b) + Esh > __float_as_int(ub.z))) != 0ull)
                                    c_blk_violation++;
#endif
                                if (vp_ != 0ull) {
                                    FS_TRIP_FAILED(a, tp_, ua.z, wv)
                                    break;
                                }
                                z2 = (f2){ub.x, ub.y};
                                c += 2;
                                FS_STEP_ARITH(w2, z2, tq_, c_)
                                FS_STEP_BOUND(tq_, c_, vq_, uc.z)
                                FS_STEP_FLOOR_FIRST(tq_, vq_)
                                f2 w4;
                                FS_STEP_ARITH(tq_, uq_, w4, d)
                                FS_STEP_BOUND(w4, d, vq_, ud.z)
                                FS_STEP_FLOOR(w4, vq_)
#ifdef FS_VERIFY_BLOCK_BOUND
                                if (kStats && bt_pass &&
                                    (__builtin_amdgcn_ballot_w64(__float_as_int(mx_c_) + Esh > __float_as_int(uc.z)) |
                                     __builtin_amdgcn_ballot_w64(__float_as_int(mx_d) + Esh > __float_as_int(ud.z))) != 0ull)
                                    c_blk_violation++;
#endif
                                if (vq_ != 0ull) {
                                    FS_TRIP_FAILED(c_, tq_, uc.z, w2)
                                    break;
                                }
                                cs += 4;
                                wv = w4, mxS = mx_d, zS = (f2){ud.x, ud.y}, pwi = __float_as_int(ud.w);
                                FS_CYC(cyc_tested += __builtin_readcyclecounter() - cyc_t4);
                                if (cs >= rl) {
                                    c = cs, wO = wv, failed = false;
                                    break;
                                }
                            }
                            }
                        } else {
                            const uint32_t lane_off = (ref + 1) * 16u;
                            const float4 *zp = zs;
                            f3 ent_a, ent_b, ent_c_, ent_d;
// ... 281 lines not shown
            {
                uint32_t lane_e;
                asm volatile("v_mbcnt_lo_u32_b32 %0, -1, 0\n\tv_mbcnt_hi_u32_b32 %0, -1, %0" : "=v"(lane_e));
                lane_cost = iterations - s_it0[wave_in_block * 64u + lane_e];
            }
        } else {
            lane_cost = la_cost;
        }
        {
            uint32_t lane_e;
            asm volatile("v_mbcnt_lo_u32_b32 %0, -1, 0\n\tv_mbcnt_hi_u32_b32 %0, -1, %0" : "=v"(lane_e));
            store_iter(A.out, A.frame, tile_y * 8u + (lane_e >> 3), tile_x * 8u + (lane_e & 7u), iterations);
        }
    }
    if (A.tile_cost && tile_x < A.tiles_x) {
        for (int off = 32; off > 0; off >>= 1) {
            const uint32_t o = __shfl_down(lane_cost, off);
            lane_cost = o > lane_cost ? o : lane_cost;
        }
        uint32_t lane_e;
        asm volatile("v_mbcnt_lo_u32_b32 %0, -1, 0\n\tv_mbcnt_hi_u32_b32 %0, -1, %0" : "=v"(lane_e));
        if (lane_e == 0u)
            A.tile_cost[tile_y * A.tiles_x + tile_x] = lane_cost;
    }
#ifdef FS_TRACE_WAVES
    if (kStats && A.stats) {
        uint64_t steps = c_pt;
        for (int off = 32; off > 0; off >>= 1) {
            const uint64_t o = __shfl_down(steps, off);
            steps = o > steps ? o : steps;
        }
        if ((threadIdx.x & 63) == 0) {
            uint32_t hw_id, xcc_id;
            asm volatile("s_getreg_b32 %0, hwreg(HW_REG_HW_ID)" : "=s"(hw_id));
            asm volatile("s_getreg_b32 %0, hwreg(HW_REG_XCC_ID)" : "=s"(xcc_id));
            const uint64_t wave = ((uint64_t)blockIdx.y * gridDim.x + blockIdx.x) * (blockDim.x >> 6) + (threadIdx.x >> 6);
            uint64_t *t = A.stats + 16 + 4 * wave;
            t[0] = trace_t0;
            t[1] = wall_clock64();
            t[2] = ((uint64_t)xcc_id << 32) | hw_id;
            t[3] = steps;
        }
    }
#endif
#ifdef FS_PROFILE_CYCLES
    if (kStats) {
        if ((threadIdx.x & 63) == 0) {
            atomicAdd((unsigned long long *)&A.stats[0], (unsigned long long)cyc_loop);
            atomicAdd((unsigned long long *)&A.stats[1], (unsigned long long)cyc_run);
            atomicAdd((unsigned long long *)&A.stats[3], (unsigned long long)cyc_body);
            atomicAdd((unsigned long long *)&A.stats[24], (unsigned long long)cyc_asm);
            atomicAdd((unsigned long long *)&A.stats[25], (unsigned long long)cyc_tested);
            atomicAdd((unsigned long long *)&A.stats[26], (unsigned long long)cyc_hot);
            atomicAdd((unsigned long long *)&A.stats[27], (unsigned long long)wall_loop);
        }
        c_at = c_la = c_px = 0;
    }
#endif
    if (kStats) {
        add_stats(A.stats, c_at, c_la, c_pt, c_px);
        for (int off = 32; off > 0; off >>= 1) {
            c_careful += __shfl_down(c_careful, off);
            c_scaled += __shfl_down(c_scaled, off);
            c_runs += __shfl_down(c_runs, off);
            const uint32_t bf = __shfl_down(c_blk_free, off), bt = __shfl_down(c_blk_tested, off);
            c_blk_free = bf > c_blk_free ? bf : c_blk_free;
            c_blk_tested = bt > c_blk_tested ? bt : c_blk_tested;
            const uint32_t cp = __shfl_down(c_pass, off), cg = __shfl_down(c_generic, off);
            c_pass = cp > c_pass ? cp : c_pass;
            c_generic = cg > c_generic ? cg : c_generic;
            const uint32_t we = __shfl_down(c_wentry, off), ws = __shfl_down(c_wstart, off), wh = __shfl_down(c_wshort, off);
            c_wentry = we > c_wentry ? we : c_wentry;
            c_wstart = ws > c_wstart ? ws : c_wstart;
            c_wshort = wh > c_wshort ? wh : c_wshort;
            const uint32_t ls = __shfl_down(c_lane_steps, off), lr = __shfl_down(c_lane_runs, off);
            c_lane_steps = ls > c_lane_steps ? ls : c_lane_steps;
            c_lane_runs = lr > c_lane_runs ? lr : c_lane_runs;
            const uint32_t ns = __shfl_down(c_nd_steps, off), nf = __shfl_down(c_nd_fail, off);
            c_nd_steps = ns > c_nd_steps ? ns : c_nd_steps;
            c_nd_fail = nf > c_nd_fail ? nf : c_nd_fail;
            const uint32_t nr = __shfl_down(c_nd_replayed, off), nm = __shfl_down(c_nd_mismatch, off);
            c_nd_replayed = nr > c_nd_replayed ? nr : c_nd_replayed;
            c_nd_mismatch = nm > c_nd_mismatch ? nm : c_nd_mismatch;
            const uint32_t bv = __shfl_down(c_blk_violation, off);
            c_blk_violation = bv > c_blk_violation ? bv : c_blk_violation;
            for (int i = 0; i < 4; i++) {
                const uint32_t y = __shfl_down(c_why[i], off);
                c_why[i] = y > c_why[i] ? y : c_why[i];
                const uint32_t y2 = __shfl_down(c_nz[i], off);
                c_nz[i] = y2 > c_nz[i] ? y2 : c_nz[i];
            }
        }
        if ((threadIdx.x & 63) == 0) {
            atomicAdd((unsigned long long *)&A.stats[5], (unsigned long long)c_careful);
            atomicAdd((unsigned long long *)&A.stats[6], (unsigned long long)c_scaled);
            atomicAdd((unsigned long long *)&A.stats[7], (unsigned long long)c_runs);
            atomicAdd((unsigned long long *)&A.stats[8], (unsigned long long)c_blk_free);
            atomicAdd((unsigned long long *)&A.stats[9], (unsigned long long)c_blk_tested);
            atomicAdd((unsigned long long *)&A.stats[10], (unsigned long long)c_pass);
            atomicAdd((unsigned long long *)&A.stats[11], (unsigned long long)c_generic);
            atomicAdd((unsigned long long *)&A.stats[12], (unsigned long long)c_wentry);
            atomicAdd((unsigned long long *)&A.stats[13], (unsigned long long)c_wstart);
            atomicAdd((unsigned long long *)&A.stats[14], (unsigned long long)c_wshort);
            atomicAdd((unsigned long long *)&A.stats[15], (unsigned long long)c_blk_violation);
            for (int i = 0; i < 4; i++) {
                atomicAdd((unsigned long long *)&A.stats[16 + i], (unsigned long long)c_why[i]);
                atomicAdd((unsigned long long *)&A.stats[20 + i], (unsigned long long)c_nz[i]);
            }
            atomicAdd((unsigned long long *)&A.stats[28], (unsigned long long)c_lane_steps);
            atomicAdd((unsigned long long *)&A.stats[29], (unsigned long long)c_lane_runs);
            atomicAdd((unsigned long long *)&A.stats[30], (unsigned long long)c_nd_steps);
            atomicAdd((unsigned long long *)&A.stats[32], (unsigned long long)c_nd_fail);
            atomicAdd((unsigned long long *)&A.stats[33], (unsigned long long)c_nd_mismatch);
            atomicAdd((unsigned long long *)&A.stats[34], (unsigned long long)c_nd_replayed);
        }
    }
}
#undef FS_CYC

static dim3 tile_grid(const FsFrame &f) { return dim3((f.width + 31) / 32, (f.local_rows + 7) / 8, 1); }

uint32_t fsk_lav2_hdr32_slots(const FsFrame &f)
{
    return ((f.width + 31u) / 32u) * 4u * ((f.local_rows + 7u) / 8u);
}

void fsk_lav2_hdr32(const FsLav2Args32 &A, int mode, bool stats, int variant, hipStream_t s)
{
    const bool lds_orbit = (variant & FS_VARIANT_FLAG_LDS_ORBIT) != 0;
    variant &= FS_VARIANT_BASE_MASK;
    const dim3 b(256), g = tile_grid(A.frame);
#define FS_LAUNCH_FAST(M, SC, LDS)                                                                                  \
    if (stats) {                                                                                                    \
        if (gs)                                                                                                     \
            hipLaunchKernelGGL((k_lav2_hdr32_fast<M, true, SC, LDS, true>), g, b, 0, s, A);                         \
        else                                                                                                        \
            hipLaunchKernelGGL((k_lav2_hdr32_fast<M, true, SC, LDS, false>), g, b, 0, s, A);                        \
    } else {                                                                                                        \
        if (gs)                                                                                                     \
            hipLaunchKernelGGL((k_lav2_hdr32_fast<M, false, SC, LDS, true>), g, b, 0, s, A);                        \
        else                                                                                                        \
            hipLaunchKernelGGL((k_lav2_hdr32_fast<M, false, SC, LDS, false>), g, b, 0, s, A);                       \
    }
#define FS_LAUNCH(M)                                                                                                \
    do {                                                                                                            \
        if (variant == FS_VARIANT_LITERAL) {                                                                        \
            fsk_lav2_lit32(A, M, stats, g, b, s);                       \
        } else {                                                                                                    \
            const bool gs = A.parity == FS_PARITY_GPUSTAGE;                                                         \
            if (variant == FS_VARIANT_TUNED_NOSCALE) {                                                              \
                FS_LAUNCH_FAST(M, false, false)                                                                     \
            } else if (lds_orbit) {                                                                                 \
                FS_LAUNCH_FAST(M, true, true)                                                                       \
            } else {                                                                                                \
                FS_LAUNCH_FAST(M, true, false)                                                                      \
            }                                                                                                       \
        }                                                                                                           \
    } while (0)
    if (mode == FS_MODE_FULL)
        FS_LAUNCH(FS_MODE_FULL);
    else if (mode == FS_MODE_PO)
        FS_LAUNCH(FS_MODE_PO);
    else
        FS_LAUNCH(FS_MODE_LAO);
#undef FS_LAUNCH
#undef FS_LAUNCH_FAST
}
```

fractalshark_amd/csrc/renderer_inputs.cpp:

```cpp
#include "renderer_state.hpp"

#include <cstddef>

using namespace fsr;

namespace {

constexpr uint64_t kQuietSlack = 32;
constexpr uint64_t quiet_orbit_units(uint64_t n)
{
    return 2 * (n + 2) + 16 + ((n + 2) + kQuietSlack + 1) / 2 + ((n + 2) + kQuietSlack);
}

hipError_t make_quiet_orbit(fs_renderer *r, uint64_t n)
{
    (void)r_release(r, r->zq);
    const uint64_t m = n + 2, slack = kQuietSlack;
    const uint64_t units = quiet_orbit_units(n);
    hipError_t err = r_alloc(r, (void **)&r->zq, units * sizeof(float4), kInput);
    if (err != hipSuccess)
        return err;
    r->zq_n = m;
    r->zs2 = (float2 *)(r->zq + 2 * m + 16);
    r->zqb = r->zq + 2 * m + 16 + (m + slack + 1) / 2;
    err = hipMemsetAsync(r->zs2, 0, ((m + slack + 1) / 2 + (m + slack)) * sizeof(float4), r->compute);
    if (err != hipSuccess)
        return err;
    fsk_make_quiet_orbit(r->zref, r->zq, r->zs2, r->zqb, m, r->compute);
    return hipGetLastError();
}

constexpr size_t kBlaPtrTableBytes = 64 * sizeof(void *);

void bla_release(fs_renderer *r)
{
    buf_release(r, r->bla_native);
    buf_release(r, r->bla_heap);
    buf_release(r, r->bla_block);
    r->bla_native_ok = r->bla_heap_ok = false;
    r->bla_level_mem.clear();
    r->bla_level_sizes.clear();
    r->bla_levels_dev = nullptr;
    r->bla_n_levels = 0;
}

hipError_t bla_layout(fs_renderer *r, const uint64_t *sizes, int32_t n_levels, size_t rec_bytes)
{
    if (n_levels > 64)
        return hipErrorInvalidValue;
    size_t total = kBlaPtrTableBytes;
    for (int32_t l = 0; l < n_levels; l++)
        total += (sizes[l] * rec_bytes + 255u) & ~(size_t)255u;
    r->bla_n_levels = 0;
    if (!r->bla_block.p || r->bla_block.cap < total) {
        bla_release(r);
        const hipError_t e = buf_reserve(r, r->bla_block, total, kInput);
        if (e != hipSuccess)
            return e;
    }
    r->bla_level_mem.assign((size_t)n_levels, nullptr);
    r->bla_level_sizes.assign((size_t)n_levels, 0);
    size_t at = kBlaPtrTableBytes;
    for (int32_t l = 0; l < n_levels; l++) {
        if (sizes[l] == 0)
            continue;
        r->bla_level_mem[(size_t)l] = r->bla_block.as<char>() + at;
        r->bla_level_sizes[(size_t)l] = sizes[l];
        at += (sizes[l] * rec_bytes + 255u) & ~(size_t)255u;
    }
    r->bla_levels_dev = (const void **)r->bla_block.p;
    return hipMemcpyAsync(r->bla_block.p, r->bla_level_mem.data(), sizeof(void *) * (size_t)n_levels, hipMemcpyHostToDevice,
                          r->compute);
}

void orbit_changed(fs_renderer *r)
{
    r->bla_native_ok = false;
    r->bla_native_stale = r->bla_n_levels > 0 && r->bla_type == FS_T_HDR32;
}

void drop_seq(fs_renderer *r)
{
    (void)r_release(r, r->wp_raw);
    r->orbit_seq = false;
}

}

namespace fsr {

hipError_t la_reserve(fs_renderer *r, size_t las_bytes, size_t stages_bytes)
{
    const hipError_t e = buf_reserve(r, r->las, las_bytes, kInput);
    return e != hipSuccess ? e : buf_reserve(r, r->stages, stages_bytes, kInput);
}

uint32_t bla_make_native(fs_renderer *r, int32_t n_levels)
{
    r->bla_native_ok = false;
    r->bla_native_stale = false;
    if (n_levels <= 2 || n_levels > kBlaMaxLevels || r->bla_type != FS_T_HDR32 || !r->orbit_ok ||
        r->orbit_type != FS_T_HDR32 || !r->zref)
        return 0;
    uint64_t total = 0;
    for (int32_t l = 2; l < n_levels; l++) {
        r->bla_level_off[l] = (uint32_t)total;
        total += r->bla_level_sizes[(size_t)l];
    }
    if (total == 0 || total > 0xFFFFFFF0ull)
        return 0;
    const uint32_t n_kmax = (uint32_t)(r->orbit_uncompressed / 4u) + 2u;
// ... 634 lines not shown
```

fractalshark_amd/csrc/renderer_launch.cpp:

```cpp
#include "renderer_state.hpp"

#include <cmath>
#include <cstdlib>

using namespace fsr;

namespace {

FsFrame make_frame(const fs_renderer *r)
{
    FsFrame f;
    f.width = r->width;
    f.height = r->height;
    f.rounded_width = r->w_block * 16u;
    f.local_rows = r->local_rows;
    f.band_first = r->band_first;
    f.band_rows = r->band_rows;
    f.band_stride = r->band_stride;
    f.iter_u64 = r->iter_bytes == 8 ? 1u : 0u;
    f.wide = (r->variant & FS_VARIANT_FLAG_WIDE) != 0 ? 1u : 0u;
    return f;
}

constexpr uint64_t kTileProbeDivisor = 32;
// ... 132 lines not shown
    const uint32_t n = (uint32_t)buffer_elems(f);
    r->pix_valid = false;
    if (buf_reserve(r, {{&r->pix_order, (size_t)n * sizeof(uint32_t)}, {&r->pix_work, (size_t)n * 2 * sizeof(uint32_t)},
                        {&r->pix_temp, fsk_pixel_order_temp_bytes(n)}}, kFrame, &r->pix_valid) != hipSuccess ||
        fsk_pixel_order_build(cost ? cost : (const uint32_t *)r->iters(), n, r->pix_work.as<uint32_t>(), r->pix_order.as<uint32_t>(),
                              r->pix_temp.p, r->pix_temp.cap, r->compute) != hipSuccess) {
        (void)hipGetLastError();
        return;
    }
    r->pix_key = key;
    r->pix_valid = true;
}

static const uint32_t *cold_tile_order(fs_renderer *r, FsTileSampleArgs &S)
{
    static const bool off = [] { const char *e = getenv("FSMI355_COLD_TILE_ORDER"); return e && e[0] == '0'; }();
    if (off || !pix_order_wanted(r, S.frame) || S.StepLength == 0u)
        return nullptr;
    S.tiles_x = (S.frame.width + 7u) / 8u, S.tiles_y = (S.frame.local_rows + 7u) / 8u;
    S.n_slots = ((S.frame.width + 31u) / 32u) * S.tiles_y * 4u;
    const size_t words = (size_t)S.n_slots * sizeof(uint32_t);
    if (buf_reserve(r, {{&r->cold_cost, words}, {&r->cold_order, words}, {&r->cold_work, 2 * words},
                        {&r->cold_temp, fsk_pixel_order_temp_bytes(S.n_slots)}}, kFrame) != hipSuccess) {
        (void)hipGetLastError();
        return nullptr;
    }
    S.cost = r->cold_cost.as<uint32_t>();
    fsk_at_tile_sample64(S, r->compute);
    if (fsk_pixel_order_build(S.cost, S.n_slots, r->cold_work.as<uint32_t>(), r->cold_order.as<uint32_t>(), r->cold_temp.p,
                              r->cold_temp.cap, r->compute) != hipSuccess) {
        (void)hipGetLastError();
        return nullptr;
    }
    fsk_tile_order_finish(r->cold_order.as<uint32_t>(), S.n_slots, S.tiles_x * S.tiles_y, r->compute);
    r->last_cold_ordered = true;
    return r->cold_order.as<uint32_t>();
}

static void fill_tile_sample(FsTileSampleArgs &S, const FsFrame &frame, const FsCoordsT<double> &coords, uint32_t n_iterations,
                             uint32_t step_length, fs::hreal<double> ThresholdC, fs::hreal<double> SqrEscapeRadius,
                             fs::hcplx<double> RefC, fs::hcplx<double> CCoeff)
{
    memset(&S, 0, sizeof(S));
    S.frame = frame;
    S.coords = coords;
    S.ThresholdC = ThresholdC, S.SqrEscapeRadius = SqrEscapeRadius;
    S.RefC = RefC, S.CCoeff = CCoeff;
    S.StepLength = step_length, S.n_iterations = n_iterations;
}


static uint32_t lav2_seq(fs_renderer *r, int type_tag, int mode, int parity, const void *coords, uint64_t n_iterations, bool wide)
{
    const bool wide_pos = wide || r->la_u64 || r->orbit_uncompressed > 0xFFFFFFFFull || r->orbit_period > 0xFFFFFFFFull;
    TimedLaunch t(r);
    auto launch = [&](auto f, const auto &at, const auto &c_low) {
        using F = decltype(f);
        FsLav2ArgsT<F> A;
        fill_lav2<F>(r, A, coords, n_iterations, parity);
        A.frame.wide |= wide_pos ? 1u : 0u;
        r->last_launch_wide = A.frame.wide != 0u;
        A.at = at;
        A.wp = r->wp_raw, A.n_wp = (uint32_t)r->orbit_size;
        A.cxLow = c_low[0], A.cyLow = c_low[1];
        if constexpr (sizeof(F) == 4)
            fsk_lav2_seq(&A, nullptr, kernel_mode(mode), r->stats_on, r->compute);
        else
            fsk_lav2_seq(nullptr, &A, kernel_mode(mode), r->stats_on, r->compute);
    };
    if (type_tag == FS_T_HDR32)
        launch(0.0f, r->at, r->c_low32);
    else
        launch(0.0, r->at64, r->c_low64);
    return (uint32_t)hipGetLastError();
}

template <class Args> static void set_orbit_hdr32(const fs_renderer *r, Args &A)
{
    A.zref = r->zref;
    A.zq = r->zq;
    A.zs = r->zq + r->zq_n;
    A.zs2 = r->zs2;
    A.zqb = r->zqb;
}

static uint32_t lav2_wide(fs_renderer *r, int type_tag, int mode, int parity, const void *coords, uint64_t n_iterations)
{
    TimedLaunch t(r);
    if (type_tag == FS_T_HDR32) {
        FsLav2ArgsT<float> A;
        fill_lav2<float>(r, A, coords, n_iterations, parity);
        set_orbit_hdr32(r, A);
        A.at = r->at;
        fsk_lav2_wide(&A, nullptr, kernel_mode(mode), r->stats_on, r->compute);
    } else {
        FsLav2ArgsT<double> A;
        fill_lav2<double>(r, A, coords, n_iterations, parity);
        A.zref = r->zref64;
        A.at = r->at64;
        fsk_lav2_wide(nullptr, &A, kernel_mode(mode), r->stats_on, r->compute);
    }
    return (uint32_t)hipGetLastError();
}

static uint32_t lav2_plain(fs_renderer *r, int type_tag, int mode, const void *coords, uint64_t n_iterations)
{
    FsLav2ArgsPlain A;
    init_args(r, A, n_iterations);
    r->last_launch_wide = A.frame.wide != 0u || r->orbit_seq;
    A.las = r->las.p;
    A.stages = r->stages.as<fs_la_stage_u32>();
    memcpy(A.coords, coords, type_tag == FS_T_F32 ? 4 * sizeof(float) : 4 * sizeof(double));
    memcpy(A.at, r->at_plain, sizeof(A.at));
    A.orbit_count = (uint32_t)r->orbit_uncompressed;
    A.stage_count = r->n_stages;
    A.la_valid = (r->la_ok && r->la_type == type_tag) ? r->la_valid : 0;
    A.use_at = r->use_at;
    if (r->orbit_seq) {
        A.wp = r->wp_raw;
        A.n_wp = (uint32_t)r->orbit_size;
        memcpy(A.c_low[0], r->c_low_plain[0], 8);
        memcpy(A.c_low[1], r->c_low_plain[1], 8);
    } else {
        A.orbit = type_tag == FS_T_F64 ? (const void *)r->orbit_f64 : (const void *)r->orbit_plain;
    }
    TimedLaunch t(r);
    fsk_lav2_plain(A, type_tag == FS_T_F32 ? 0 : (type_tag == FS_T_F64 ? 1 : 2), kernel_mode(mode), r->stats_on, r->compute);
    return (uint32_t)hipGetLastError();
}

static uint32_t lav2_2x32(fs_renderer *r, int mode, const void *coords, uint64_t n_iterations)
{
    FsLav2Args2x32 A;
    init_args(r, A, n_iterations);
    r->last_launch_wide = A.frame.wide != 0u || r->orbit_seq;
    A.las = r->las.as<const fs_la_2x32_u32>();
    A.stages = r->stages.as<fs_la_stage_u32>();
    memcpy(A.coords, coords, sizeof(A.coords));
    A.at = r->at2x32;
    A.orbit_count = (uint32_t)r->orbit_uncompressed;
    A.stage_count = r->n_stages;
    A.la_valid = (r->la_ok && r->la_type == FS_T_HDR2X32) ? r->la_valid : 0;
    A.use_at = r->use_at;
    if (r->orbit_seq) {
        A.wp = (const fs_orbit_2x32_rc *)r->wp_raw;
        A.n_wp = (uint32_t)r->orbit_size;
        memcpy(&A.cxLow, r->c_low_plain[0], sizeof(fs_real_2x32));
        memcpy(&A.cyLow, r->c_low_plain[1], sizeof(fs_real_2x32));
    } else {
        A.orbit = r->orbit_2x32;
    }
    const fs_renderer::PixKey pk = pix_key_of(r, A.frame, FS_T_HDR2X32, mode, 0, coords, sizeof(A.coords), n_iterations);
    A.pixel_order = r->orbit_seq ? nullptr : pix_order_for(r, A.frame, pk);
    const bool second = !r->orbit_seq && A.pixel_order == nullptr && pix_second_sighting(r, A.frame, pk);
    A.pixel_cost = second ? pix_cost_for(r, A.frame, false) : nullptr;
    {
        TimedLaunch t(r);
        if (!r->orbit_seq && A.pixel_order == nullptr && !second && mode != FS_LAV2_PO && A.use_at && A.la_valid) {
            auto R = [](const fs_real_2x32 &x) { return fs::hreal<double>{(double)x.head + (double)x.tail, x.e}; };
            auto Cx = [](const fs_cplx_2x32 &c) {
                return fs::hcplx<double>{(double)c.re_head + (double)c.re_tail, (double)c.im_head + (double)c.im_tail, c.e};
            };
            FsTileSampleArgs S;
            fill_tile_sample(S, A.frame, FsCoordsT<double>{R(A.coords[0]), R(A.coords[1]), R(A.coords[2]), R(A.coords[3])},
                             A.n_iterations, A.at.StepLength, R(A.at.ThresholdC), R(A.at.SqrEscapeRadius), Cx(A.at.RefC),
                             Cx(A.at.CCoeff));
// ... 352 lines not shown

uint32_t fs_set_kernel_variant(fs_renderer *r, int variant)
{
    const int base = variant & FS_VARIANT_BASE_MASK, flags = variant & ~FS_VARIANT_BASE_MASK;
    if (base > FS_VARIANT_TUNED_NOSCALE ||
        (flags & ~(FS_VARIANT_FLAG_LDS_ORBIT | FS_VARIANT_FLAG_REFILL | FS_VARIANT_FLAG_WIDE | FS_VARIANT_FLAG_NATURAL_ORDER |
                   FS_VARIANT_FLAG_BLA_POOL)) != 0)
        return hipErrorInvalidValue;
    r->variant = base | flags;
    return 0;
}

uint32_t fs_forget_tile_costs(fs_renderer *r)
{
    r->lav2_cost_valid = false;
    r->po_order_valid = false;
    r->pix_valid = false;
    r->pix_seen = false;
    r->at_order_valid = false;
    return 0;
}

int fs_last_frame_tile_ordered(fs_renderer *r) { return r->last_frame_ordered ? 1 : 0; }
int fs_last_frame_sampled_tile_order(fs_renderer *r) { return r->last_cold_ordered ? 1 : 0; }

uint32_t fs_read_tile_costs(fs_renderer *r, uint32_t *out, uint64_t max_words, uint64_t *n_tiles)
{
    if (uint32_t e = use_device(r))
        return e;
    if (!r->lav2_cost.p || !r->lav2_cost_valid)
        return FS_ERR_6;
    const uint64_t n = (uint64_t)((r->lav2_cost_key.width + 7u) / 8u) * ((r->lav2_cost_key.local_rows + 7u) / 8u);
    if (n_tiles)
        *n_tiles = n;
    const uint64_t m = n < max_words ? n : max_words;
    if (out && m) {
        FS_TRY(hipMemcpyAsync(out, r->lav2_cost.p, m * sizeof(uint32_t), hipMemcpyDeviceToHost, r->compute));
        FS_TRY(hipStreamSynchronize(r->compute));
    }
    return 0;
}

uint32_t fs_seq_cursor_probe(fs_renderer *r, int wide_positions, uint64_t start, uint32_t n, void *out)
{
    if (uint32_t e = use_device(r))
        return e;
    if (!r->orbit_ok || !r->orbit_seq || !r->wp_raw || !out)
        return FS_ERR_6;
    const bool is64 = r->orbit_type == FS_T_HDR64;
    const size_t rec = is64 ? sizeof(fs::hcplx<double>) : sizeof(fs::hcplx<float>);
    void *dev = nullptr;
    FS_TRY(r_alloc(r, &dev, (size_t)n * rec, kFrame));
    fsk_seq_cursor_probe(is64, wide_positions != 0, r->wp_raw, (uint32_t)r->orbit_size,
                         is64 ? (const void *)&r->c_low64[0] : (const void *)&r->c_low32[0],
                         is64 ? (const void *)&r->c_low64[1] : (const void *)&r->c_low32[1], start, n, dev, r->compute);
    hipError_t err = hipGetLastError();
    if (err == hipSuccess)
        err = hipMemcpyAsync(out, dev, (size_t)n * rec, hipMemcpyDeviceToHost, r->compute);
    if (err == hipSuccess)
        err = hipStreamSynchronize(r->compute);
    (void)r_free(r, dev);
    return (uint32_t)err;
}

uint32_t fs_read_tile_order(fs_renderer *r, uint32_t *out, uint64_t max_words)
{
    if (uint32_t e = use_device(r))
        return e;
    if (!r->lav2_order.p || !r->lav2_last_ordered)
        return FS_ERR_6;
    const uint64_t n = (uint64_t)((r->lav2_cost_key.width + 7u) / 8u) * ((r->lav2_cost_key.local_rows + 7u) / 8u);
    const uint64_t m = n < max_words ? n : max_words;
    FS_TRY(hipMemcpyAsync(out, r->lav2_order.p, m * sizeof(uint32_t), hipMemcpyDeviceToHost, r->compute));
    FS_TRY(hipStreamSynchronize(r->compute));
    return 0;
}

uint32_t fs_enable_step_count(fs_renderer *r, int enable)
{
    r->stats_on = enable != 0;
    return 0;
}

uint32_t fs_test_block_threshold(fs_renderer *r, const int32_t *bound_bits, const int32_t *scale_shift, const int32_t *dc_bits,
                                 int32_t *threshold_out, uint32_t n)
{
    if (!r || !bound_bits || !scale_shift || !dc_bits || !threshold_out)
        return (uint32_t)hipErrorInvalidValue;
    if (n == 0)
        return 0;
    FS_TRY(hipSetDevice(r->device));
    int *d = nullptr;
    FS_TRY(hipMalloc((void **)&d, (size_t)n * 4 * sizeof(int)));
    uint32_t rc = (uint32_t)hipMemcpy(d, bound_bits, n * sizeof(int), hipMemcpyHostToDevice);
    if (!rc)
        rc = (uint32_t)hipMemcpy(d + n, scale_shift, n * sizeof(int), hipMemcpyHostToDevice);
    if (!rc)
        rc = (uint32_t)hipMemcpy(d + 2 * (size_t)n, dc_bits, n * sizeof(int), hipMemcpyHostToDevice);
    if (!rc) {
        fsk_test_block_threshold(d, d + n, d + 2 * (size_t)n, d + 3 * (size_t)n, n, r->compute);
        rc = (uint32_t)hipGetLastError();
    }
    if (!rc)
        rc = (uint32_t)hipStreamSynchronize(r->compute);
    if (!rc)
        rc = (uint32_t)hipMemcpy(threshold_out, d + 3 * (size_t)n, n * sizeof(int), hipMemcpyDeviceToHost);
    hipFree(d);
    return rc;
}

uint32_t fs_read_stats_raw(fs_renderer *r, uint64_t *out, uint64_t max_words)
{
    if (uint32_t e = use_device(r))
        return e;
    if (!r->stats)
        return FS_ERR_6;
    const size_t n = r->stats_words < max_words ? r->stats_words : (size_t)max_words;
    FS_TRY(hipMemcpyAsync(out, r->stats, n * sizeof(uint64_t), hipMemcpyDeviceToHost, r->compute));
    FS_TRY(hipStreamSynchronize(r->compute));
    return 0;
}

uint32_t fs_read_step_count(fs_renderer *r, uint64_t counts[8])
{
    if (uint32_t e = use_device(r))
        return e;
    if (!r->stats)
        return FS_ERR_6;
    if (r->last_launch_wide)
        return FS_ERR_UNSUPPORTED;
    FS_TRY(hipMemcpyAsync(counts, r->stats, 8 * sizeof(uint64_t), hipMemcpyDeviceToHost, r->compute));
    FS_TRY(hipStreamSynchronize(r->compute));
    return 0;
}

}
```

fractalshark_amd/csrc/renderer_state.hpp:

```cpp
#pragma once
#include <hip/hip_runtime.h>

#include <cstring>
#include <initializer_list>
#include <mutex>
#include <vector>

#include "../../include/fsmi355_internal.h"
#include "kernels.h"

#define FS_TRY(expr)                                                                                                  \
    do {                                                                                                              \
        hipError_t e_ = (expr);                                                                                       \
        if (e_ != hipSuccess)                                                                                         \
            return (uint32_t)e_;                                                                                      \
    } while (0)

struct DevBuf {
    void *p = nullptr;
    size_t cap = 0;
    template <class T> T *as() const { return (T *)p; }
};

struct fs_renderer {
    int device = 0;
    hipStream_t compute = nullptr;
    hipStream_t display = nullptr;
    static constexpr uint32_t kTimingRing = 64;
    hipEvent_t ev_start[kTimingRing] = {}, ev_stop[kTimingRing] = {};
    hipEvent_t ev_mid[kTimingRing] = {};
    bool mid_valid[kTimingRing] = {};
    uint64_t timed_launches = 0;

    uint32_t width = 0, height = 0, aa = 0, iter_bytes = 0;
    uint32_t w_block = 0, h_block = 0;
    uint32_t color_w = 0, color_h = 0;
    size_t n_cu = 0, n_color_cu = 0;
    uint32_t band_first = 0, band_rows = 0, band_stride = 0;
    uint32_t local_rows = 0, local_rows_padded = 0;

    DevBuf iters_internal;
    void *iters_external = nullptr;
    size_t iters_external_bytes = 0;
    fs_reduction reduce_seed{};
    fs_color16 *colors = nullptr;
    fs_reduction *reduction = nullptr;
    uint64_t *stats = nullptr;
    size_t stats_words = 40;

    uint32_t *queue = nullptr;
    DevBuf tile_probe, tile_order;
    DevBuf lav2_cost, lav2_order, lav2_sort_tmp;
    bool lav2_cost_valid = false;
    struct CostKey {
        uint32_t width, local_rows, band_first, band_rows, band_stride;
        uint64_t orbit_gen;
        bool operator==(const CostKey &o) const
        {
            return width == o.width && local_rows == o.local_rows && band_first == o.band_first && band_rows == o.band_rows &&
                   band_stride == o.band_stride && orbit_gen == o.orbit_gen;
        }
    } lav2_cost_key{};
    bool po_order_valid = false;
    CostKey po_order_key{};
    uint64_t po_order_epoch = 0, po_order_iterations = 0;
    unsigned char po_order_coords[32] = {};
    bool last_frame_ordered = false;
    DevBuf at_res, at_cost, at_order;
    bool at_order_valid = false;
    DevBuf pix_cost;
    DevBuf pix_order, pix_work, pix_temp;
    bool pix_valid = false;
    bool pix_seen = false;
    struct PixKey {
        uint32_t rounded_width, local_rows, band_first, band_rows, band_stride;
        int type_tag, mode, parity;
        uint64_t orbit_gen, orbit_epoch, n_iterations;
        unsigned char coords[64];
        bool operator==(const PixKey &o) const { return memcmp(this, &o, sizeof(*this)) == 0; }
    } pix_key{}, pix_seen_key{}, at_key{};
    DevBuf cold_cost, cold_order, cold_work, cold_temp;
    bool last_cold_ordered = false;
    bool lav2_last_ordered = false;
    bool last_launch_wide = false;
    bool stats_on = false;
    int variant = FS_VARIANT_TUNED;

    fs_color16 *pal = nullptr;
    uint32_t pal_iters = 0, pal_aux_depth = 0;
    const fs_color16 *pal_cached_host = nullptr;
    uint64_t pal_cached_gen = 0;

    uint64_t orbit_gen = 0;
    uint64_t orbit_epoch = 0, orbit_fp = 0, pending_fp = 0;
    bool orbit_ok = false;
    int orbit_type = -1;
    fs_orbit_2x32 *orbit_2x32 = nullptr;
    int scaled_type = -1;
    void *scaled_t = nullptr;
    fs_orbit_f32_bad *scaled_f = nullptr;
    uint64_t scaled_count = 0;
    float4 *zref = nullptr;
    float4 *zq = nullptr;
    uint64_t zq_n = 0;
    float2 *zs2 = nullptr;
    float4 *zqb = nullptr;
    FsZ64 *zref64 = nullptr;
    fs_orbit_f64 *orbit_f64 = nullptr;
    void *orbit_plain = nullptr;
    alignas(8) uint8_t at_plain[sizeof(fs_at_f64_u32)] = {0};
    uint64_t orbit_size = 0, orbit_uncompressed = 0, orbit_period = 0;
    int compressed_mode = 0;
    bool orbit_seq = false;
    void *wp_raw = nullptr;
    fs_real_hdr32 c_low32[2] = {};
    fs_real_hdr64 c_low64[2] = {};
    alignas(8) uint8_t c_low_plain[2][16] = {};

    uint64_t la_gen = 0;
    bool la_ok = false;
    int la_type = -1;
    DevBuf las;
    DevBuf stages;
    uint32_t n_las = 0, n_stages = 0;
    int la_valid = 0, use_at = 0;
    bool la_u64 = false;
    uint32_t at_step_hi = 0;
    fs_at_hdr32_u32 at{};
    fs_at_hdr64_u32 at64{};
    fs_at_2x32_u32 at2x32{};

    std::vector<void *> bla_level_mem;
    std::vector<uint64_t> bla_level_sizes;
    const void **bla_levels_dev = nullptr;
    int bla_type = -1;
    int32_t bla_n_levels = 0, bla_lm2 = 0;

    DevBuf cx_row;

    std::vector<void *> host_allocs;
    struct Block {
        void *p;
        size_t bytes;
    };
    std::vector<Block> live_blocks, kept_blocks;
    std::mutex kept_mu;
    size_t host_alloc_bytes = 0;
    uint32_t feature_slice = 0;
    uint32_t exact_slice = 0;
    bool exact_no_compaction = false;
    uint64_t exact_stats[4] = {};
    uint32_t az_gather_rows = 0;
    FsAzStats az_seed{};
    bool inject_input_oom = false;
    DevBuf arena;
    uint32_t *la_mail = nullptr;
    uint32_t la_mail_seq = 0;
    DevBuf bla_block;
    DevBuf bla_native;
    bool bla_native_ok = false;
    bool bla_native_stale = false;
    uint32_t bla_native_total = 0;
    DevBuf bla_heap;
    bool bla_heap_ok = false;
    uint64_t bla_heap_positions = 0;
    uint32_t bla_heap_nq = 0;
    uint32_t bla_level_off[kBlaMaxLevels] = {0};

    void *iters() const { return iters_external ? iters_external : iters_internal.p; }
    bool memory_initialized() const { return iters() != nullptr && width != 0; }
};

namespace fsr {

uint32_t use_device(const fs_renderer *r);

uint32_t ensure_streams(fs_renderer *r);

enum AllocKind { kFrame = 0, kInput = 1 };

hipError_t r_alloc(fs_renderer *r, void **out, size_t bytes, AllocKind kind);
template <class T> hipError_t r_alloc(fs_renderer *r, T **out, size_t bytes, AllocKind kind)
{
    return r_alloc(r, (void **)out, bytes, kind);
}

hipError_t r_free(fs_renderer *r, const void *cp);

template <class T> hipError_t r_release(fs_renderer *r, T *&p)
// ... 55 lines not shown
```

fractalshark_amd/csrc/scaled_runs.hpp:

```cpp
#pragma once

#include <hip/hip_runtime.h>
#include <stdint.h>

#include "hdr_math.hpp"
#include "kernels.h"

namespace {

static __device__ __forceinline__ float fs_max_abs(float a, float b)
{
    float r;
    asm("v_max_f32_e64 %0, |%1|, |%2|" : "=v"(r) : "v"(a), "v"(b));
    return r;
}
static __device__ __forceinline__ float fs_min_abs(float a, float b)
{
    float r;
    asm("v_min_f32_e64 %0, |%1|, |%2|" : "=v"(r) : "v"(a), "v"(b));
    return r;
}

}

// ... 76 lines not shown
    if (kStats && __builtin_amdgcn_ballot_w64(!(fs_min_abs(NW_.x, NW_.y) >= 0x1p-56f)) != 0ull) \
        c_blk_violation++;
#else
#define FS_STEP_FLOOR_FIRST(NW_, V) FS_STEP_FLOOR(NW_, V)
#endif
#define FS_FAST_LOOP_FL(PF)                                                                                           \
    asm volatile(                                                                                                   \
        ".Lfl_loop_%=:\n\t"  \
        "v_max_i32_e32 v62, v60, %[imdc]\n\t"                                                                       \
        "s_cmp_gt_u32 %[off], %[lim8]\n\t"                                                                          \
        "v_add_u32_e32 v62, v62, %[esh]\n\t"                                                                        \
        "s_cbranch_scc1 .Lfl_out_%=\n\t"                                                                            \
        "v_cmp_lt_i32_e64 %[m], s67, v62\n\t" FS_FL_H                                                               \
        "s_or_b64 %[m], %[m], vcc\n\t"                                                                              \
        "s_cbranch_scc1 .Lfl_out_%=\n\t"            \
        FS_PK_F(FS_R0, "s[64:65]") "s_mov_b32 %[eb], s62\n\t"                                                       \
        "s_load_dwordx16 s[36:51], s[68:69], %[off]\n\t"                                                            \
        "s_load_dwordx16 s[52:67], s[68:69], %[off] offset:0x40\n\t"                                                \
        FS_PK_MA(FS_R0) FS_FL_N1("v54", "v55") FS_PK_MB(FS_R0) FS_FL_N2("v48", "v49") FS_PK_P FS_FL_C FS_PK_A(FS_R1) \
        "s_waitcnt lgkmcnt(0)\n\t" PF                                                                               \
        FS_PK_F(FS_R1, "s[36:37]") FS_PK_MA(FS_R1) FS_PK_MB(FS_R1) FS_PK_P                                          \
        "s_cbranch_vccnz .Lfl_fp_%=\n\t" FS_PK_A(FS_R2)  \
        FS_PK_F(FS_R2, "s[40:41]") FS_FL_N1("v50", "v51") FS_PK_MA(FS_R2) FS_PK_MB(FS_R2) FS_FL_N2("v52", "v53")    \
        FS_PK_P FS_FL_C FS_PK_A(FS_R3)                                                                              \
        FS_PK_F(FS_R3, "s[44:45]") FS_PK_MA(FS_R3) FS_PK_MB(FS_R3) FS_PK_P                                          \
        "s_cbranch_vccnz .Lfl_f1_%=\n\t" FS_PK_A(FS_R0)  \
        FS_PK_F(FS_R0, "s[48:49]") FS_FL_N1("v54", "v55") FS_PK_MA(FS_R0) FS_PK_MB(FS_R0) FS_FL_N2("v48", "v49")    \
        FS_PK_P FS_FL_C FS_PK_A(FS_R1) FS_T_X("v48", "v49")                                                         \
        FS_PK_F(FS_R1, "s[52:53]") FS_PK_MA(FS_R1) FS_PK_MB(FS_R1) FS_PK_P                                          \
        "s_cbranch_vccnz .Lfl_f2_%=\n\t"  \
        "v_max_i32_e32 v62, v60, %[imdc]\n\t" FS_PK_A(FS_R2) "v_add_u32_e32 v62, v62, %[esh]\n\t"                   \
                                                         \
        FS_PK_F(FS_R2, "s[56:57]") "v_cmp_lt_i32_e64 %[m], s51, v62\n\t" FS_FL_H FS_PK_MA(FS_R2)                    \
        "s_or_b64 %[m], %[m], vcc\n\t" FS_PK_MB(FS_R2) FS_PK_P "s_cbranch_scc1 .Lfl_blk_%=\n\t" FS_PK_A(FS_R3)      \
        FS_FL_N1("v50", "v51")                                                                                      \
        FS_PK_F(FS_R3, "s[60:61]") FS_FL_N2("v52", "v53") FS_PK_MA(FS_R3) FS_PK_MB(FS_R3) FS_FL_C FS_PK_P           \
        "s_cbranch_vccnz .Lfl_f3_%=\n\t" FS_PK_A(FS_R0)                                                             \
        "s_add_u32 %[off], %[off], 0x80\n\t"  \
        FS_T_X("v48", "v49") "s_branch .Lfl_loop_%=\n"                                                              \
        ".Lfl_out_%=:\n\t"  \
        "s_mov_b32 %[eb], s62\n\t" FS_FL_N1("v54", "v55") FS_FL_N2("v48", "v49") FS_FL_C                            \
        "s_cbranch_vccnz .Lfl_fp_%=\n\t"                                                                            \
        "s_mov_b32 %[st], 0\n\t"                                                                                    \
        "s_branch .Lfl_end_%=\n"                                                                                    \
        ".Lfl_blk_%=:\n\t"                        \
        "s_mov_b32 %[st], 0\n\t"                                                                                    \
        "s_mov_b64 s[64:65], s[48:49]\n\t"                                                                          \
        "s_mov_b32 s67, s51\n\t"                                                                                    \
        "s_add_u32 %[off], %[off], 0x40\n\t"                                                                        \
        "s_branch .Lfl_end_%=\n"                                                                                    \
        ".Lfl_fp_%=:\n\t"             \
        "s_mov_b32 %[st], 2\n\t"                                                                                    \
        "s_sub_u32 %[off], %[off], 0x20\n\t"                                                                        \
        "s_branch .Lfl_end_%=\n"                                                                                    \
        ".Lfl_f1_%=:\n\t"                                                                                           \
        "s_mov_b32 %[st], 1\n\t"                                                                                    \
        "s_mov_b32 %[eb], s38\n\t"                                                                                  \
        "s_branch .Lfl_end_%=\n"                                                                                    \
        ".Lfl_f2_%=:\n\t"                                                                                           \
        "s_mov_b32 %[st], 2\n\t"                                                                                    \
        "s_mov_b32 %[eb], s46\n\t"                                                                                  \
        "s_add_u32 %[off], %[off], 0x20\n\t"                                                                        \
        "s_branch .Lfl_end_%=\n"                                                                                    \
        ".Lfl_f3_%=:\n\t"                                                                                           \
        "s_mov_b32 %[st], 1\n\t"                                                                                    \
        "s_mov_b32 %[eb], s54\n\t"                                                                                  \
        "s_add_u32 %[off], %[off], 0x40\n"                                                                          \
        ".Lfl_end_%=:\n\t"                                                                                          \
        "s_waitcnt lgkmcnt(0)"         \
        : "+{v[48:49]}"(wv), "={v[50:51]}"(r1), "={v[52:53]}"(r2), "+{v[54:55]}"(r3), "={v[56:57]}"(ts_),           \
          "={v[58:59]}"(ta_), "+{v60}"(mxS), "={v61}"(tn_), "={v62}"(tl_), [m] "=&s"(msk_), [st] "=&s"(st),         \
          [eb] "=&s"(ebo), "+{s67}"(pwi), "+{s[64:65]}"(zS), [off] "+s"(off), [pf] "=&s"(pf_), [pg] "=&s"(pg_),     \
          [ph] "=&s"(ph_), [xa] "+s"(xacc_)                                                                         \
        : [se] "v"(sE2), [dc] "v"(dcs), [esh] "v"(Esh), [imdc] "v"(imdc), [lim8] "s"(lim8), "{s[68:69]}"(zpb),      \
          [flr] "s"(kFloorBits), [flr56] "s"((127 - 56) << 23)                                                      \
        : "s36", "s37", "s38", "s39", "s40", "s41", "s42", "s43", "s44", "s45", "s46", "s47", "s48", "s49", "s50",  \
          "s51", "s52", "s53", "s54", "s55", "s56", "s57", "s58", "s59", "s60", "s61", "s62", "s63", "s66", "vcc",  \
          "scc")

#define FS_FL_ACC(A, B) "v_min3_f32 v61, |" A "|, |" B "|, v61\n\t"
#define FS_BT_DC_MAX "v_max_i32_e32 v62, v60, %[imdc]\n\t"
#define FS_BT_DC_ADD "v_add_u32_e32 v62, v62, %[esh]\n\t"

#define FS_BT_T(BW)                                                                                                 \
    "s_sub_i32 %[t], " BW ", %[eshm]\n\t"                                                                           \
    "s_cselect_b32 %[t], 0x46800000, %[t]\n\t"                                                                      \
    "s_min_i32 %[t], %[t], 0x46800000\n\t"                                                                          \
    "s_cmp_gt_i32 %[sdc], " BW "\n\t"                                                                               \
    "s_cselect_b32 %[t], -1, %[t]\n\t"
#define FS_BT_V "v_cmp_lt_i32_e32 vcc, %[t], v60\n\t"
#define FS_PK_PN(NW) "v_pk_add_f32 " NW ", v[58:59], v[56:57] neg_lo:[0,1] neg_hi:[0,0]\n\t"
#define FS_FDU_LOOP(L, PF, PRE, POST)                                                                               \
        ".L" L "_loop_%=:\n\t"       \
        "s_cmp_gt_u32 %[off], %[lim8]\n\t"                                                                          \
        "s_cbranch_scc1 .L" L "_out_%=\n\t"                                                                         \
        "s_cbranch_vccnz .L" L "_out_%=\n\t"                                                      \
        FS_PK_F(FS_R0, "s[64:65]")                                                                                  \
        "s_load_dwordx16 s[36:51], s[68:69], %[off]\n\t"                                                            \
        "s_load_dwordx16 s[52:67], s[68:69], %[off] offset:0x40\n\t"                                                \
        FS_PK_MA(FS_R0) FS_PK_MB(FS_R0) PRE POST(FS_R1)                                                             \
        "s_waitcnt lgkmcnt(0)\n\t" PF FS_BT_T("s51")                                                                \
        FS_PK_F(FS_R1, "s[36:37]") FS_FL_ACC("v50", "v51") FS_PK_MA(FS_R1) FS_PK_MB(FS_R1) PRE POST(FS_R2)          \
        FS_PK_F(FS_R2, "s[40:41]") FS_FL_ACC("v52", "v53") FS_PK_MA(FS_R2) FS_PK_MB(FS_R2) PRE POST(FS_R3)          \
        FS_PK_F(FS_R3, "s[44:45]") FS_FL_ACC("v54", "v55") FS_PK_MA(FS_R3) FS_PK_MB(FS_R3) PRE POST(FS_R0)          \
         \
        FS_PK_F(FS_R0, "s[48:49]") FS_FL_ACC("v48", "v49") FS_PK_MA(FS_R0) FS_T_X("v48", "v49") FS_PK_MB(FS_R0)     \
        PRE POST(FS_R1)                                                                                             \
        FS_PK_F(FS_R1, "s[52:53]") FS_BT_V FS_PK_MA(FS_R1) FS_PK_MB(FS_R1) PRE                                      \
        "s_cbranch_vccnz .L" L "_blk_%=\n\t" POST(FS_R2)                                                            \
        FS_PK_F(FS_R2, "s[56:57]") FS_FL_ACC("v50", "v51") FS_PK_MA(FS_R2) FS_FL_ACC("v52", "v53") FS_PK_MB(FS_R2)  \
        PRE POST(FS_R3)                                                                                             \
        FS_PK_F(FS_R3, "s[60:61]") FS_FL_ACC("v54", "v55") FS_PK_MA(FS_R3) FS_PK_MB(FS_R3) PRE POST(FS_R0)          \
        "s_add_u32 %[off], %[off], 0x80\n\t" FS_BT_T("s67")                                                         \
        FS_T_X("v48", "v49") FS_FL_ACC("v48", "v49") FS_BT_V "s_branch .L" L "_loop_%=\n"                           \
        ".L" L "_blk_%=:\n\t"        \
        "s_mov_b64 s[64:65], s[48:49]\n\t"                                                                          \
        "s_mov_b32 s67, s51\n\t"                                                                                    \
        "s_add_u32 %[off], %[off], 0x40\n"                                                                          \
        ".L" L "_out_%=:\n\t"
#define FS_FAST_LOOP_FDU(PF)                                                                                        \
    asm volatile(                                                                                                   \
        "v_mov_b32_e32 v61, 0x7f800000\n\t" FS_BT_T("s67") FS_BT_V                                                  \
        "s_cmp_lg_u32 %[nd], 0\n\t"                                                                                 \
        "s_cbranch_scc1 .Lfn_loop_%=\n"                                                                             \
        FS_FDU_LOOP("fu", PF, FS_PK_P, FS_PK_A)                \
        "s_mov_b32 %[st], 0\n\t" FS_FL_C                                                                            \
        "s_cbranch_vccz .Lfu_end_%=\n\t"                                                                            \
        "s_mov_b32 %[st], 3\n\t"                                                                                    \
        "s_branch .Lfu_end_%=\n"                                                                                    \
        FS_FDU_LOOP("fn", PF, "", FS_PK_PN)             \
        "v_max_f32_e64 v62, |%[dcx]|, |%[dcy]|\n\t"                                                                 \
        "s_mov_b32 %[st], 0\n\t"                                                                                    \
        "v_ldexp_f32 v62, v62, 26\n\t"                                                                              \
        "v_max_f32_e32 v62, %[flr], v62\n\t"                                                                        \
        "v_cmp_gt_f32_e32 vcc, v62, v61\n\t"                                                                        \
        "s_cbranch_vccz .Lfu_end_%=\n\t"  \
        "s_mov_b32 %[st], 5\n\t" FS_FL_C                                                                            \
        "s_cbranch_vccz .Lfu_end_%=\n\t"                                                                            \
        "s_mov_b32 %[st], 3\n"                                                                                      \
        ".Lfu_end_%=:\n\t"                                                                                        \
        "s_waitcnt lgkmcnt(0)"                                                                                      \
        : "+{v[48:49]}"(wv), "={v[50:51]}"(r1), "={v[52:53]}"(r2), "={v[54:55]}"(r3), "={v[56:57]}"(ts_),           \
          "={v[58:59]}"(ta_), "+{v60}"(mxS), "={v61}"(tn_), "={v62}"(tl_), [t] "=&s"(bt_t_), [st] "=&s"(st),        \
          "+{s67}"(pwi), "+{s[64:65]}"(zS), [off] "+s"(off), [pf] "=&s"(pf_), [pg] "=&s"(pg_), [ph] "=&s"(ph_)      \
        : [se] "v"(sE2), [dc] "v"(dcs), [dcx] "v"(dcs.x), [dcy] "v"(dcs.y), [eshm] "s"(Esh_cap),                    \
          [sdc] "s"(sdc_bits), [lim8] "s"(lim8), [nd] "s"(nd_sel), "{s[68:69]}"(zpb), [flr] "s"(kFloorBits)         \
        : "s36", "s37", "s38", "s39", "s40", "s41", "s42", "s43", "s44", "s45", "s46", "s47", "s48", "s49", "s50",  \
          "s51", "s52", "s53", "s54", "s55", "s56", "s57", "s58", "s59", "s60", "s61", "s62", "s63", "s66", "vcc",  \
          "scc")
constexpr uint32_t kNdBackoffEntry = 8;
constexpr uint32_t kNdBackoffVerdict = 32;

#define FS_FD16_TAIL(EC, ED)                                                                                        \
    FS_PK_F(FS_R2, EC) FS_FL_ACC("v50", "v51") FS_PK_MA(FS_R2) FS_FL_ACC("v52", "v53") FS_PK_MB(FS_R2)              \
    FS_PK_P FS_PK_A(FS_R3)                                                                                          \
    FS_PK_F(FS_R3, ED) FS_FL_ACC("v54", "v55") FS_PK_MA(FS_R3) FS_PK_MB(FS_R3) FS_PK_P FS_PK_A(FS_R0)

#define FS_FD16D_PAIR(EA, EB_, BW, WAIT, LOADS)                                                                     \
    FS_PK_F(FS_R0, EA) FS_FL_ACC("v48", "v49") FS_PK_MA(FS_R0)                                                      \
    "v_max3_f32 v62, |v48|, |v49|, %[imdc]\n\t"                                                                     \
    FS_PK_MB(FS_R0) FS_PK_P                                                                                         \
    "v_subrev_u32_e32 v45, 0x46800000, v62\n\t"                                                                     \
    FS_PK_A(FS_R1)                                                                                                  \
    "v_add_u32_e32 v62, v62, %[esh]\n\t" WAIT                                                                       \
    FS_PK_F(FS_R1, EB_)                                                                                             \
    "v_sub_i32 v62, v62, " BW " clamp\n\t"                                                                          \
    FS_PK_MA(FS_R1)                                                                                                 \
    "v_max3_i32 v63, v63, v62, v45\n\t"                                                                             \
    FS_PK_MB(FS_R1) FS_PK_P LOADS FS_PK_A(FS_R2)
#define FS_FAST_LOOP_FD16P                                                                                          \
    asm volatile(                                                                                                   \
        "v_mov_b32_e32 v61, 0x7f800000\n\t"  \
        "v_bfrev_b32_e32 v63, 1\n\t"                                                                                \
        "s_lshr_b32 %[oc], %[off], 1\n\t"                                                                           \
        "s_load_dwordx16 s[36:51], s[68:69], %[oc]\n\t"                                                             \
        "s_load_dwordx2 s[72:73], s[70:71], %[off]\n"                                                               \
        ".Lfp_loop_%=:\n\t"  \
        "v_sub_u32_e32 v45, %[flr], v61\n\t"                                                                        \
        FS_BT_DC_MAX "s_cmp_gt_u32 %[off], %[lim16]\n\t"                                                            \
        "v_max_i32_e32 v45, v45, v63\n\t"                                                                           \
        FS_BT_DC_ADD                                                                                                \
        "v_cmp_lt_i32_e32 vcc, 0, v45\n\t"                                                                          \
        "s_cbranch_vccnz .Lfp_redo_%=\n\t"                                                 \
        "s_cbranch_scc1 .Lfp_out_%=\n\t"                   \
        "v_mov_b32_e32 v46, v48\n\t"                                                                                \
        "v_mov_b32_e32 v47, v49\n\t"                                                                                \
        "s_mov_b32 %[cko], %[off]\n\t"                                                                              \
        "v_mov_b32_e32 v61, 0x7f800000\n\t"         \
        FS_PK_F(FS_R0, "s[66:67]")                                                                                  \
        "v_sub_i32 v62, v62, s75 clamp\n\t"                                                                         \
        "v_subrev_u32_e32 v45, 0x46800000, v60\n\t"                                                                 \
        "s_waitcnt lgkmcnt(0)\n\t"                      \
        "s_lshr_b32 %[oc], %[off], 1\n\t"                                                                           \
        "s_load_dwordx16 s[52:67], s[68:69], %[oc] offset:0x40\n\t"                                                 \
        "s_load_dwordx2 s[74:75], s[70:71], %[off] offset:0x8\n\t"                                                  \
        FS_PK_MA(FS_R0)                                                                                             \
        "v_max_i32_e32 v63, v62, v45\n\t"                                                                           \
        FS_PK_MB(FS_R0) FS_PK_P FS_PK_A(FS_R1)                                                                      \
        FS_PK_F(FS_R1, "s[36:37]") FS_FL_ACC("v50", "v51") FS_PK_MA(FS_R1) FS_PK_MB(FS_R1) FS_PK_P FS_PK_A(FS_R2)   \
        FS_PK_F(FS_R2, "s[38:39]") FS_FL_ACC("v52", "v53") FS_PK_MA(FS_R2) FS_PK_MB(FS_R2) FS_PK_P FS_PK_A(FS_R3)   \
        FS_PK_F(FS_R3, "s[40:41]") FS_FL_ACC("v54", "v55") FS_PK_MA(FS_R3) FS_PK_MB(FS_R3) FS_PK_P FS_PK_A(FS_R0)   \
                                                                                                  \
        FS_FD16D_PAIR("s[42:43]", "s[44:45]", "s72", "", "") FS_FD16_TAIL("s[46:47]", "s[48:49]")                   \
           \
        FS_FD16D_PAIR("s[50:51]", "s[52:53]", "s73", "s_waitcnt lgkmcnt(0)\n\t",                                    \
                      "s_load_dwordx16 s[36:51], s[68:69], %[oc] offset:0x80\n\t"                                   \
                      "s_load_dwordx2 s[72:73], s[70:71], %[off] offset:0x100\n\t")                                 \
        FS_FD16_TAIL("s[54:55]", "s[56:57]")                                                                        \
                                                                                                \
        FS_FD16D_PAIR("s[58:59]", "s[60:61]", "s74", "", "") FS_FD16_TAIL("s[62:63]", "s[64:65]")                   \
        "s_add_u32 %[off], %[off], 0x100\n\t"                                                                       \
        FS_T_X("v48", "v49") FS_FL_ACC("v48", "v49") "s_branch .Lfp_loop_%=\n"                                      \
        ".Lfp_redo_%=:\n\t"  \
        "v_mov_b32_e32 v48, v46\n\t"                                                                                \
        "v_mov_b32_e32 v49, v47\n\t"                                                                                \
        "v_cmp_lt_i32_e32 vcc, 0, v63\n\t"                                                                          \
        "s_mov_b32 %[off], %[cko]\n\t"                                                                              \
        FS_T_X("v46", "v47")                                                                                        \
        "s_mov_b32 %[st], 3\n\t"                                                                                    \
        "s_cbranch_vccz .Lfp_end_%=\n\t"                                                                            \
        "s_mov_b32 %[st], 4\n\t"                                                                                    \
        "s_branch .Lfp_end_%=\n"                                                                                    \
        ".Lfp_out_%=:\n\t"  \
        "s_mov_b32 %[st], 0\n"                                                                                      \
        ".Lfp_end_%=:\n\t"                                                                                          \
        "s_waitcnt lgkmcnt(0)"                                                                                      \
        : "+{v[48:49]}"(wv), "={v[50:51]}"(r1), "={v[52:53]}"(r2), "={v[54:55]}"(r3), "={v[56:57]}"(ts_),           \
          "={v[58:59]}"(ta_), "+{v60}"(mxS), "={v61}"(tn_), "={v62}"(tl_), "={v[46:47]}"(ck_), "={v45}"(th_),       \
          "={v63}"(va_), [st] "=&s"(st), "+{s75}"(pwi), "+{s[66:67]}"(zS), [off] "+s"(off), [oc] "=&s"(oc_),        \
          [cko] "=&s"(cko_)                                                                                         \
        : [se] "v"(sE2), [dc] "v"(dcs), [esh] "v"(Esh), [imdc] "v"(imdc), [lim16] "s"(lim16), "{s[68:69]}"(zpb2),   \
          "{s[70:71]}"(zqbp), [flr] "s"(kFloorBits)                                                                 \
// ... 92 lines not shown
```

include/fsmi355_internal.h:

```cpp
#ifndef FSMI355_INTERNAL_H
#define FSMI355_INTERNAL_H

#include "fsmi355.h"

#ifdef __cplusplus
extern "C" {
#endif

float fs_last_kernel_ms(const fs_renderer *r);
uint32_t fs_kernel_ms_history(const fs_renderer *r, float *ms_out, uint32_t n);
uint32_t fs_kernel_ms_split_history(const fs_renderer *r, float *first_ms, float *second_ms, uint32_t n);
enum { FS_VARIANT_LDS_ORBIT = 0x100, FS_VARIANT_REFILL = 0x200, FS_VARIANT_WIDE_COUNTERS = 0x400,
       FS_VARIANT_NATURAL_TILE_ORDER = 0x800, FS_VARIANT_BLA_POOL = 0x1000 };
uint32_t fs_set_kernel_variant(fs_renderer *r, int variant);
uint32_t fs_forget_tile_costs(fs_renderer *r);
int fs_last_frame_tile_ordered(fs_renderer *r);
int fs_last_frame_sampled_tile_order(fs_renderer *r);
uint32_t fs_read_tile_costs(fs_renderer *r, uint32_t *out, uint64_t max_words, uint64_t *n_tiles);
uint32_t fs_seq_cursor_probe(fs_renderer *r, int wide_positions, uint64_t start, uint32_t n, void *out);
uint32_t fs_read_tile_order(fs_renderer *r, uint32_t *out, uint64_t max_words);
uint32_t fs_set_feature_slice(fs_renderer *r, uint32_t steps);
uint32_t fs_set_autozoom_gather_cap(fs_renderer *r, uint32_t rows);
uint32_t fs_set_exact_slice(fs_renderer *r, uint32_t steps, int no_compaction);
uint32_t fs_read_exact_stats(const fs_renderer *r, uint64_t out[4]);
uint32_t fs_exact_wide_state(fs_renderer *r, uint32_t frac_bits, uint32_t limbs, const uint32_t *cx, const uint32_t *cy,
                             uint32_t n_samples, uint32_t steps, uint32_t *out_x, uint32_t *out_y);
uint32_t fs_enable_step_count(fs_renderer *r, int enable);
uint32_t fs_read_step_count(fs_renderer *r, uint64_t counts[8]);
uint32_t fs_read_stats_raw(fs_renderer *r, uint64_t *out, uint64_t max_words);
uint32_t fs_test_block_threshold(fs_renderer *r, const int32_t *bound_bits, const int32_t *scale_shift, const int32_t *dc_bits,
                                 int32_t *threshold_out, uint32_t n);
uint32_t fs_time_render_current(fs_renderer *r, uint64_t n_iterations, uint32_t repeats, float ms_out[2]);


int32_t fs_bla_num_levels(const fs_renderer *r);
int32_t fs_bla_lm2(const fs_renderer *r);
uint64_t fs_bla_level_size(const fs_renderer *r, int32_t level);
uint32_t fs_read_bla_level(fs_renderer *r, int32_t level, void *out, uint64_t max_records);
uint32_t fs_la_counts(const fs_renderer *r, uint32_t *n_las, uint32_t *n_stages, int *use_at, int *is_valid);
uint32_t fs_read_la(fs_renderer *r, void *las_out, uint32_t max_las, void *stages_out, uint32_t max_stages, void *at_out);

float fs_group_gather_ms(fs_group *g);

#ifdef __cplusplus
}
#endif

#endif
```

Baseline: 210.4 Mpix/s.

## Add precomputed 8-step no-deep-zoom bound for a lighter nd fast loop path

Precomputes a per-orbit-index bound (znz) in the quiet-orbit kernel, certifying that an 8-step block can skip per-step checks in the nd loop. The nd fast loop now loads this bound, tests it against the pixel's scaled delta, and enters a leaner NDZ loop that does eight steps with fewer checks. The cost is extra orbit-preprocessing memory and work, an extra scalar load per entry, and more complex inline assembly. Adds a test hook and a stats counter for NDZ steps.

```diff
diff --git a/fractalshark_amd/_capi.py b/fractalshark_amd/_capi.py
--- a/fractalshark_amd/_capi.py
+++ b/fractalshark_amd/_capi.py
@@ -161,6 +161,7 @@
     _decl(lib, "fs_time_render_current", u32, [vp, u64, u32, vp])
     _decl(lib, "fs_read_stats_raw", u32, [vp, vp, u64])
     _decl(lib, "fs_test_block_threshold", u32, [vp, vp, vp, vp, vp, u32])
+    _decl(lib, "fs_test_ndz_threshold", u32, [vp, vp, vp, vp, vp, u32])
     _decl(lib, "fs_build_la", u32, [vp, C.c_int, vp, C.c_int])
     _decl(lib, "fs_build_la_mt", u32, [vp, C.c_int, vp, C.c_int, C.c_int])
     _decl(lib, "fs_la_counts", u32, [vp, vp, vp, vp, vp])
@@ -212,7 +213,7 @@
     "fs_render_direct_lp", "fs_clear",
     "fs_render_current", "fs_sync_compute", "fs_compute_stream", "fs_sync_display", "fs_query_compute", "fs_enqueue_done_callback",
     "fs_host_fallback_bytes", "fs_idle_device_bytes", "fs_release_idle_device_memory", "fs_set_compressed_orbit_mode", "fs_orbit_device_bytes", "fs_get_width", "fs_get_height", "fs_last_kernel_ms", "fs_set_kernel_variant", "fs_kernel_ms_history", "fs_kernel_ms_split_history", "fs_forget_tile_costs", "fs_last_frame_tile_ordered", "fs_last_frame_sampled_tile_order", "fs_read_tile_costs", "fs_read_tile_order", "fs_seq_cursor_probe", "fs_enable_step_count", "fs_read_step_count",
-    "fs_time_render_current", "fs_read_stats_raw", "fs_test_block_threshold", "fs_build_la", "fs_build_la_mt", "fs_la_counts", "fs_read_la",
+    "fs_time_render_current", "fs_read_stats_raw", "fs_test_block_threshold", "fs_test_ndz_threshold", "fs_build_la", "fs_build_la_mt", "fs_la_counts", "fs_read_la",
     "fs_group_create", "fs_group_destroy", "fs_group_size", "fs_group_transport", "fs_group_renderer", "fs_group_init_memory",
     "fs_group_upload_orbit", "fs_group_upload_orbit_compressed", "fs_group_upload_la", "fs_group_upload_bla",
     "fs_group_upload_orbit_scaled", "fs_group_render_lav2", "fs_group_render_bla", "fs_group_render_scaled",
diff --git a/fractalshark_amd/csrc/kernels.h b/fractalshark_amd/csrc/kernels.h
--- a/fractalshark_amd/csrc/kernels.h
+++ b/fractalshark_amd/csrc/kernels.h
@@ -91,6 +91,7 @@
     const float4 *zs;
     const float2 *zs2;
     const float4 *zqb;
+    const float *znz;
     const typename FsDev<F>::LA *las;
     const fs_la_stage_u32 *stages;
     uint64_t *stats;
@@ -143,6 +144,7 @@
     const float4 *zs;
     const float2 *zs2;
     const float4 *zqb;
+    const float *znz;
     const typename FsDev<F>::BLA *const *levels;
     uint64_t *stats;
     uint32_t *queue;
@@ -301,7 +303,7 @@
 template <class F>
 void fsk_feature_direct_step(FsFeatDirectLane<F> *st, void *out, uint64_t n, int find, int iter_u64, fs::hreal<F> R,
                              uint32_t slice, uint32_t *unfinished, hipStream_t s);
-void fsk_make_quiet_orbit(const float4 *zref, float4 *zq, float2 *zs2, float4 *zqb, uint64_t n, hipStream_t s);
+void fsk_make_quiet_orbit(const float4 *zref, float4 *zq, float2 *zs2, float4 *zqb, float *znz, uint64_t n, hipStream_t s);
 void fsk_tile_order(const uint32_t *probe, uint32_t probe_pitch, uint32_t tiles_x, uint32_t tiles_y, uint32_t threshold,
                     uint32_t *order, uint32_t n_slots, hipStream_t s);
 uint32_t fsk_tile_order_work_words(uint32_t n_tiles);
@@ -471,3 +473,4 @@
                int use_small_exponents, void *at_out, uint32_t *use_at, hipStream_t s);
 void fsk_la_pack(bool is64, const void *in, void *out, uint32_t n, hipStream_t s);
 void fsk_test_block_threshold(const int *bw, const int *eshm, const int *sdc, int *t_out, uint32_t n, hipStream_t s);
+void fsk_test_ndz_threshold(const int *bw, const int *eshm, const int *sdc, int *t_out, uint32_t n, hipStream_t s);
diff --git a/fractalshark_amd/csrc/kernels.hip b/fractalshark_amd/csrc/kernels.hip
--- a/fractalshark_amd/csrc/kernels.hip
+++ b/fractalshark_amd/csrc/kernels.hip
@@ -56,10 +56,36 @@
     return ok ? best * (1.0f - 0x1p-10f) : -0.0f;
 }
 
+__device__ __forceinline__ float ndz_body_bound(const float4 *__restrict__ zref, uint64_t j, uint64_t n)
+{
+    if (j + 8 >= n)
+        return -0.0f;
+    const float b0 = scaled_block_bound(zref, j, n), b4 = scaled_block_bound(zref, j + 4, n);
+    if (__float_as_int(b0) == (int)0x80000000 || __float_as_int(b4) == (int)0x80000000)
+        return -0.0f;
+    float best = b0, grow = 1.0f;
+    bool ok = true;
+    for (uint32_t m = 0; m < 8; m++) {
+        const float4 v = zref[j + m];
+        const int e = __float_as_int(v.z);
+        const float lo = fs_min_abs(__builtin_amdgcn_ldexpf(v.x, e + 1), __builtin_amdgcn_ldexpf(v.y, e + 1));
+        ok = ok && lo >= 0x1p-100f;
+        if (m == 4)
+            best = __builtin_fminf(best, b4 / grow);
+        best = __builtin_fminf(best, lo * 0x1p-26f / grow);
+        const float mk = __builtin_amdgcn_ldexpf(fs_max_abs(v.x, v.y), e < -200 ? -200 : (e > 100 ? 100 : e));
+        grow *= (4.0f * mk + 3.8f) * (1.0f + 0x1p-10f);
+    }
+    best *= 1.0f - 0x1p-10f;
+    return ok && best >= 0x1p-120f ? best : -0.0f;
+}
+
 __global__ void k_make_quiet_orbit(const float4 *__restrict__ zref, float4 *__restrict__ zq, float2 *__restrict__ zs2,
-                                   float4 *__restrict__ zqb, uint64_t n)
+                                   float4 *__restrict__ zqb, float *__restrict__ znz, uint64_t n, uint64_t slack)
 {
     const uint64_t i = (uint64_t)blockIdx.x * blockDim.x + threadIdx.x;
+    if (i < slack)
+        znz[n + i] = -0.0f;
     if (i >= n)
         return;
     const float4 v = zref[i];
@@ -71,6 +97,7 @@
     zs2[i] = make_float2(__builtin_amdgcn_ldexpf(v.x, e + 1), __builtin_amdgcn_ldexpf(v.y, e + 1));
     zqb[i] = make_float4(scaled_block_bound(zref, i + 3, n), scaled_block_bound(zref, i + 7, n),
                          scaled_block_bound(zref, i + 11, n), scaled_block_bound(zref, i + 15, n));
+    znz[i] = ndz_body_bound(zref, i, n);
 }
 
 namespace {
@@ -642,9 +669,10 @@
     hipLaunchKernelGGL(k_prepare_orbit_hdr32, dim3((unsigned)((n + 255) / 256)), dim3(256), 0, s, in, out, n);
 }
 
-void fsk_make_quiet_orbit(const float4 *zref, float4 *zq, float2 *zs2, float4 *zqb, uint64_t n, hipStream_t s)
-{
-    hipLaunchKernelGGL(k_make_quiet_orbit, dim3((unsigned)((n + 255) / 256)), dim3(256), 0, s, zref, zq, zs2, zqb, n);
+void fsk_make_quiet_orbit(const float4 *zref, float4 *zq, float2 *zs2, float4 *zqb, float *znz, uint64_t n, hipStream_t s)
+{
+    hipLaunchKernelGGL(k_make_quiet_orbit, dim3((unsigned)((n + 255) / 256)), dim3(256), 0, s, zref, zq, zs2, zqb, znz, n,
+                       (uint64_t)32);
 }
 
 __global__ void k_decompress_orbit_hdr64(const fs_orbit_hdr64_rc *__restrict__ wp, uint64_t n_wp, uint64_t n_uncompressed,
diff --git a/fractalshark_amd/csrc/kernels_lav2_hdr32.hip b/fractalshark_amd/csrc/kernels_lav2_hdr32.hip
--- a/fractalshark_amd/csrc/kernels_lav2_hdr32.hip
+++ b/fractalshark_amd/csrc/kernels_lav2_hdr32.hip
@@ -31,6 +31,25 @@
 void fsk_test_block_threshold(const int *bw, const int *eshm, const int *sdc, int *t_out, uint32_t n, hipStream_t s)
 {
     hipLaunchKernelGGL(k_test_block_threshold, dim3(n), dim3(64), 0, s, bw, eshm, sdc, t_out, n);
+}
+
+__global__ void k_test_ndz_threshold(const int *__restrict__ bw, const int *__restrict__ eshm, const int *__restrict__ sdc,
+                                     int *__restrict__ t_out, uint32_t n)
+{
+    const uint32_t i = blockIdx.x;
+    if (i >= n)
+        return;
+    const int b = __builtin_amdgcn_readfirstlane(bw[i]), e = __builtin_amdgcn_readfirstlane(eshm[i]),
+              d = __builtin_amdgcn_readfirstlane(sdc[i]);
+    int t;
+    asm volatile("s_mov_b32 s72, %[b]\n\t" FS_BT_T2("s72") : [t] "=&s"(t) : [b] "s"(b), [eshm] "s"(e), [sdc] "s"(d) : "s72", "scc");
+    if (threadIdx.x == 0)
+        t_out[i] = t;
+}
+
+void fsk_test_ndz_threshold(const int *bw, const int *eshm, const int *sdc, int *t_out, uint32_t n, hipStream_t s)
+{
+    hipLaunchKernelGGL(k_test_ndz_threshold, dim3(n), dim3(64), 0, s, bw, eshm, sdc, t_out, n);
 }
 
 template <int Mode, bool kStats, bool kScaled, bool kLds = false, bool kGpuStage = false>
@@ -76,6 +95,7 @@
     uint32_t c_blk_free = 0, c_blk_tested = 0;
     uint32_t c_lane_steps = 0, c_lane_runs = 0;
     uint32_t c_nd_steps = 0, c_nd_fail = 0, c_nd_replayed = 0, c_nd_mismatch = 0;
+    uint32_t c_ndz_steps = 0;
 #ifdef FS_PROFILE_CYCLES
     uint64_t cyc_loop = 0, cyc_run = 0, cyc_body = 0, cyc_t0 = 0, cyc_t1 = 0, cyc_t2 = 0;
     uint64_t cyc_asm = 0, cyc_tested = 0, cyc_hot = 0, cyc_t3 = 0, cyc_t4 = 0, cyc_t5 = 0, wall_loop = 0, wall_t0 = 0;
@@ -534,6 +554,7 @@
                             const uint32_t rl = (uint32_t)__builtin_amdgcn_readfirstlane((int)run_len);
                             const uint32_t lim8 = (rl << 4) - 0x80u;
                             const float4 *const zpb = zpu;
+                            const float *const znp = A.znz + ref_u;
                             for (;;) {
 #ifdef FS_VERIFY_BLOCK_BOUND
                                 const long long bt_d = (long long)pwi - (long long)Esh_cap;
@@ -548,6 +569,7 @@
                                     float tn_, tl_;
                                     uint64_t msk_;
                                     int st, ebo, pf_, pg_, ph_, bt_t_;
+                                    uint32_t nz_ = 0;
                                     const uint32_t c_in = cs;
                                     uint32_t off = cs << 4;
                                     FS_CYC(cyc_t3 = __builtin_readcyclecounter());
@@ -560,7 +582,7 @@
                                                 const float mxS_s = mxS;
                                                 const int pwi_s = pwi;
                                                 const uint32_t off_s = off;
-                                                FS_FAST_LOOP_FDU(FS_PF_NONE);
+                                                FS_FAST_LOOP_FDU(FS_PF_NONE, FS_NDZ_COUNT);
                                                 const int st_n = __builtin_amdgcn_readfirstlane(st);
                                                 if (st_n != 5 && st_n != 3) {
                                                     const f2 wv_n = wv, zS_n = zS;
@@ -569,7 +591,9 @@
                                                     const uint32_t off_n = off;
                                                     wv = wv_s, zS = zS_s, mxS = mxS_s, pwi = pwi_s, off = off_s;
                                                     nd_sel = 0;
-                                                    FS_FAST_LOOP_FDU(FS_PF_NONE);
+                                                    const uint32_t nz_n = nz_;
+                                                    FS_FAST_LOOP_FDU(FS_PF_NONE, FS_NDZ_COUNT);
+                                                    nz_ = nz_n;
                                                     const bool lane_diff = __float_as_int(wv.x) != __float_as_int(wv_n.x) ||
                                                                            __float_as_int(wv.y) != __float_as_int(wv_n.y) ||
                                                                            __float_as_int(mxS) != __float_as_int(mxS_n);
@@ -588,7 +612,7 @@
                                                     st = st_n;
                                                 }
                                             } else {
-                                                FS_FAST_LOOP_FDU(FS_PF_NONE);
+                                                FS_FAST_LOOP_FDU(FS_PF_NONE, "");
                                             }
                                         }
                                         ebo = 0;
@@ -619,8 +643,10 @@
                                         break;
                                     }
                                     cs = (uint32_t)__builtin_amdgcn_readfirstlane((int)off) >> 4;
-                                    if (kStats && nd_form != 0)
+                                    if (kStats && nd_form != 0) {
                                         c_nd_steps += cs - c_in;
+                                        c_ndz_steps += (uint32_t)__builtin_amdgcn_readfirstlane((int)nz_);
+                                    }
                                     pwi = __builtin_amdgcn_readfirstlane(pwi);
                                     if (kStats)
                                         c_blk_free += (cs - c_in) >> 2;
@@ -1068,6 +1094,8 @@
             const uint32_t nr = __shfl_down(c_nd_replayed, off), nm = __shfl_down(c_nd_mismatch, off);
             c_nd_replayed = nr > c_nd_replayed ? nr : c_nd_replayed;
             c_nd_mismatch = nm > c_nd_mismatch ? nm : c_nd_mismatch;
+            const uint32_t nzs = __shfl_down(c_ndz_steps, off);
+            c_ndz_steps = nzs > c_ndz_steps ? nzs : c_ndz_steps;
             const uint32_t bv = __shfl_down(c_blk_violation, off);
             c_blk_violation = bv > c_blk_violation ? bv : c_blk_violation;
             for (int i = 0; i < 4; i++) {
@@ -1099,6 +1127,7 @@
             atomicAdd((unsigned long long *)&A.stats[32], (unsigned long long)c_nd_fail);
             atomicAdd((unsigned long long *)&A.stats[33], (unsigned long long)c_nd_mismatch);
             atomicAdd((unsigned long long *)&A.stats[34], (unsigned long long)c_nd_replayed);
+            atomicAdd((unsigned long long *)&A.stats[35], (unsigned long long)c_ndz_steps);
         }
     }
 }
diff --git a/fractalshark_amd/csrc/renderer_inputs.cpp b/fractalshark_amd/csrc/renderer_inputs.cpp
--- a/fractalshark_amd/csrc/renderer_inputs.cpp
+++ b/fractalshark_amd/csrc/renderer_inputs.cpp
@@ -9,7 +9,7 @@
 constexpr uint64_t kQuietSlack = 32;
 constexpr uint64_t quiet_orbit_units(uint64_t n)
 {
-    return 2 * (n + 2) + 16 + ((n + 2) + kQuietSlack + 1) / 2 + ((n + 2) + kQuietSlack);
+    return 2 * (n + 2) + 16 + ((n + 2) + kQuietSlack + 1) / 2 + ((n + 2) + kQuietSlack) + ((n + 2) + kQuietSlack + 3) / 4;
 }
 
 hipError_t make_quiet_orbit(fs_renderer *r, uint64_t n)
@@ -23,10 +23,11 @@
     r->zq_n = m;
     r->zs2 = (float2 *)(r->zq + 2 * m + 16);
     r->zqb = r->zq + 2 * m + 16 + (m + slack + 1) / 2;
+    r->znz = (float *)(r->zqb + (m + slack));
     err = hipMemsetAsync(r->zs2, 0, ((m + slack + 1) / 2 + (m + slack)) * sizeof(float4), r->compute);
     if (err != hipSuccess)
         return err;
-    fsk_make_quiet_orbit(r->zref, r->zq, r->zs2, r->zqb, m, r->compute);
+    fsk_make_quiet_orbit(r->zref, r->zq, r->zs2, r->zqb, r->znz, m, r->compute);
     return hipGetLastError();
 }
 
diff --git a/fractalshark_amd/csrc/renderer_launch.cpp b/fractalshark_amd/csrc/renderer_launch.cpp
--- a/fractalshark_amd/csrc/renderer_launch.cpp
+++ b/fractalshark_amd/csrc/renderer_launch.cpp
@@ -238,6 +238,7 @@
     A.zs = r->zq + r->zq_n;
     A.zs2 = r->zs2;
     A.zqb = r->zqb;
+    A.znz = r->znz;
 }
 
 static uint32_t lav2_wide(fs_renderer *r, int type_tag, int mode, int parity, const void *coords, uint64_t n_iterations)
@@ -756,8 +757,23 @@
     return 0;
 }
 
+static uint32_t test_threshold(fs_renderer *r, const int32_t *bound_bits, const int32_t *scale_shift, const int32_t *dc_bits,
+                               int32_t *threshold_out, uint32_t n, bool ndz);
+
 uint32_t fs_test_block_threshold(fs_renderer *r, const int32_t *bound_bits, const int32_t *scale_shift, const int32_t *dc_bits,
                                  int32_t *threshold_out, uint32_t n)
+{
+    return test_threshold(r, bound_bits, scale_shift, dc_bits, threshold_out, n, false);
+}
+
+uint32_t fs_test_ndz_threshold(fs_renderer *r, const int32_t *bound_bits, const int32_t *scale_shift, const int32_t *dc_bits,
+                               int32_t *threshold_out, uint32_t n)
+{
+    return test_threshold(r, bound_bits, scale_shift, dc_bits, threshold_out, n, true);
+}
+
+static uint32_t test_threshold(fs_renderer *r, const int32_t *bound_bits, const int32_t *scale_shift, const int32_t *dc_bits,
+                               int32_t *threshold_out, uint32_t n, bool ndz)
 {
     if (!r || !bound_bits || !scale_shift || !dc_bits || !threshold_out)
         return (uint32_t)hipErrorInvalidValue;
@@ -772,7 +788,10 @@
     if (!rc)
         rc = (uint32_t)hipMemcpy(d + 2 * (size_t)n, dc_bits, n * sizeof(int), hipMemcpyHostToDevice);
     if (!rc) {
-        fsk_test_block_threshold(d, d + n, d + 2 * (size_t)n, d + 3 * (size_t)n, n, r->compute);
+        if (ndz)
+            fsk_test_ndz_threshold(d, d + n, d + 2 * (size_t)n, d + 3 * (size_t)n, n, r->compute);
+        else
+            fsk_test_block_threshold(d, d + n, d + 2 * (size_t)n, d + 3 * (size_t)n, n, r->compute);
         rc = (uint32_t)hipGetLastError();
     }
     if (!rc)
diff --git a/fractalshark_amd/csrc/renderer_state.hpp b/fractalshark_amd/csrc/renderer_state.hpp
--- a/fractalshark_amd/csrc/renderer_state.hpp
+++ b/fractalshark_amd/csrc/renderer_state.hpp
@@ -105,6 +105,7 @@
     uint64_t zq_n = 0;
     float2 *zs2 = nullptr;
     float4 *zqb = nullptr;
+    float *znz = nullptr;
     FsZ64 *zref64 = nullptr;
     fs_orbit_f64 *orbit_f64 = nullptr;
     void *orbit_plain = nullptr;
diff --git a/fractalshark_amd/csrc/scaled_runs.hpp b/fractalshark_amd/csrc/scaled_runs.hpp
--- a/fractalshark_amd/csrc/scaled_runs.hpp
+++ b/fractalshark_amd/csrc/scaled_runs.hpp
@@ -182,22 +182,49 @@
 #define FS_BT_DC_MAX "v_max_i32_e32 v62, v60, %[imdc]\n\t"
 #define FS_BT_DC_ADD "v_add_u32_e32 v62, v62, %[esh]\n\t"
 
-#define FS_BT_T(BW)                                                                                                 \
+#define FS_BT_TH(BW, HB)                                                                                            \
     "s_sub_i32 %[t], " BW ", %[eshm]\n\t"                                                                           \
-    "s_cselect_b32 %[t], 0x46800000, %[t]\n\t"                                                                      \
-    "s_min_i32 %[t], %[t], 0x46800000\n\t"                                                                          \
+    "s_cselect_b32 %[t], " HB ", %[t]\n\t"                                                                          \
+    "s_min_i32 %[t], %[t], " HB "\n\t"                                                                              \
     "s_cmp_gt_i32 %[sdc], " BW "\n\t"                                                                               \
     "s_cselect_b32 %[t], -1, %[t]\n\t"
+#define FS_BT_T(BW) FS_BT_TH(BW, "0x46800000")
 #define FS_BT_V "v_cmp_lt_i32_e32 vcc, %[t], v60\n\t"
 #define FS_PK_PN(NW) "v_pk_add_f32 " NW ", v[58:59], v[56:57] neg_lo:[0,1] neg_hi:[0,0]\n\t"
-#define FS_FDU_LOOP(L, PF, PRE, POST)                                                                               \
+#define FS_NDZ_HZ "0x3d000000"
+#define FS_BT_T2(BW) FS_BT_TH(BW, FS_NDZ_HZ)
+#define FS_PK_ZA(W, Z) "v_pk_mul_f32 v[58:59], " W ", " Z " op_sel_hi:[0,1]\n\t"
+#define FS_PK_ZB(W, Z) "v_pk_mul_f32 v[56:57], " W ", " Z " op_sel:[1,1] op_sel_hi:[1,0]\n\t"
+#define FS_NDZ_STEP(W, WA, WB, Z, NW) FS_PK_ZA(W, Z) FS_FL_ACC(WA, WB) FS_PK_ZB(W, Z) FS_PK_PN(NW)
+#define FS_NDZ_LOAD                                                                                                 \
+    "s_lshr_b32 %[t], %[off], 2\n\t"                                                                                \
+    "s_load_dword s72, s[70:71], %[t] offset:0x20\n\t"
+#define FS_FDU_TAIL(L) FS_BT_T("s67") FS_T_X("v48", "v49") FS_FL_ACC("v48", "v49") FS_BT_V "s_branch .L" L "_loop_%=\n"
+#define FS_NDZ_TAIL                                                                                                 \
+    FS_BT_T2("s72") FS_T_X("v48", "v49") FS_FL_ACC("v48", "v49") FS_BT_V                                            \
+    "s_cbranch_vccz .Lfz_loop_%=\n\t" FS_BT_T("s67") FS_BT_V "s_branch .Lfn_loop_%=\n"
+#define FS_NDZ_LOOP(PF, CNT)                                                                                        \
+        ".Lfz_loop_%=:\n\t"                                                                                         \
+        "s_cmp_gt_u32 %[off], %[lim8]\n\t"                                                                          \
+        "s_cbranch_scc1 .Lfn_out_%=\n\t"                                                                            \
+        FS_PK_ZA(FS_R0, "s[64:65]") FS_PK_ZB(FS_R0, "s[64:65]")                                                     \
+        "s_load_dwordx16 s[36:51], s[68:69], %[off]\n\t"                                                            \
+        "s_load_dwordx16 s[52:67], s[68:69], %[off] offset:0x40\n\t"                                                \
+        FS_NDZ_LOAD FS_PK_PN(FS_R1) CNT                                                                             \
+        "s_waitcnt lgkmcnt(0)\n\t" PF                                                                               \
+        FS_NDZ_STEP(FS_R1, "v50", "v51", "s[36:37]", FS_R2) FS_NDZ_STEP(FS_R2, "v52", "v53", "s[40:41]", FS_R3)     \
+        FS_NDZ_STEP(FS_R3, "v54", "v55", "s[44:45]", FS_R0) FS_NDZ_STEP(FS_R0, "v48", "v49", "s[48:49]", FS_R1)     \
+        FS_NDZ_STEP(FS_R1, "v50", "v51", "s[52:53]", FS_R2) FS_NDZ_STEP(FS_R2, "v52", "v53", "s[56:57]", FS_R3)     \
+        FS_NDZ_STEP(FS_R3, "v54", "v55", "s[60:61]", FS_R0)                                                         \
+        "s_add_u32 %[off], %[off], 0x80\n\t" FS_NDZ_TAIL
+#define FS_FDU_LOOP(L, PF, PRE, POST, XLOAD, TAIL)                                                                  \
         ".L" L "_loop_%=:\n\t"       \
         "s_cmp_gt_u32 %[off], %[lim8]\n\t"                                                                          \
         "s_cbranch_scc1 .L" L "_out_%=\n\t"                                                                         \
         "s_cbranch_vccnz .L" L "_out_%=\n\t"                                                      \
         FS_PK_F(FS_R0, "s[64:65]")                                                                                  \
         "s_load_dwordx16 s[36:51], s[68:69], %[off]\n\t"                                                            \
-        "s_load_dwordx16 s[52:67], s[68:69], %[off] offset:0x40\n\t"                                                \
+        "s_load_dwordx16 s[52:67], s[68:69], %[off] offset:0x40\n\t" XLOAD                                          \
         FS_PK_MA(FS_R0) FS_PK_MB(FS_R0) PRE POST(FS_R1)                                                             \
         "s_waitcnt lgkmcnt(0)\n\t" PF FS_BT_T("s51")                                                                \
         FS_PK_F(FS_R1, "s[36:37]") FS_FL_ACC("v50", "v51") FS_PK_MA(FS_R1) FS_PK_MB(FS_R1) PRE POST(FS_R2)          \
@@ -211,24 +238,31 @@
         FS_PK_F(FS_R2, "s[56:57]") FS_FL_ACC("v50", "v51") FS_PK_MA(FS_R2) FS_FL_ACC("v52", "v53") FS_PK_MB(FS_R2)  \
         PRE POST(FS_R3)                                                                                             \
         FS_PK_F(FS_R3, "s[60:61]") FS_FL_ACC("v54", "v55") FS_PK_MA(FS_R3) FS_PK_MB(FS_R3) PRE POST(FS_R0)          \
-        "s_add_u32 %[off], %[off], 0x80\n\t" FS_BT_T("s67")                                                         \
-        FS_T_X("v48", "v49") FS_FL_ACC("v48", "v49") FS_BT_V "s_branch .L" L "_loop_%=\n"                           \
+        "s_add_u32 %[off], %[off], 0x80\n\t" TAIL                                                                   \
         ".L" L "_blk_%=:\n\t"        \
         "s_mov_b64 s[64:65], s[48:49]\n\t"                                                                          \
         "s_mov_b32 s67, s51\n\t"                                                                                    \
         "s_add_u32 %[off], %[off], 0x40\n"                                                                          \
         ".L" L "_out_%=:\n\t"
-#define FS_FAST_LOOP_FDU(PF)                                                                                        \
+#define FS_NDZ_COUNT "s_add_u32 %[nz], %[nz], 8\n\t"
+#define FS_FAST_LOOP_FDU(PF, CNT)                                                                                   \
     asm volatile(                                                                                                   \
         "v_mov_b32_e32 v61, 0x7f800000\n\t" FS_BT_T("s67") FS_BT_V                                                  \
         "s_cmp_lg_u32 %[nd], 0\n\t"                                                                                 \
-        "s_cbranch_scc1 .Lfn_loop_%=\n"                                                                             \
-        FS_FDU_LOOP("fu", PF, FS_PK_P, FS_PK_A)                \
+        "s_cbranch_scc1 .Lfz_entry_%=\n"                                                                            \
+        FS_FDU_LOOP("fu", PF, FS_PK_P, FS_PK_A, "", FS_FDU_TAIL("fu"))  \
         "s_mov_b32 %[st], 0\n\t" FS_FL_C                                                                            \
         "s_cbranch_vccz .Lfu_end_%=\n\t"                                                                            \
         "s_mov_b32 %[st], 3\n\t"                                                                                    \
         "s_branch .Lfu_end_%=\n"                                                                                    \
-        FS_FDU_LOOP("fn", PF, "", FS_PK_PN)             \
+        ".Lfz_entry_%=:\n\t"  \
+        "s_lshr_b32 %[t], %[off], 2\n\t"                                                                            \
+        "s_load_dword s72, s[70:71], %[t]\n\t"                                                                      \
+        "s_waitcnt lgkmcnt(0)\n\t" FS_BT_T2("s72") FS_BT_V                                                          \
+        "s_cbranch_vccz .Lfz_loop_%=\n\t" FS_BT_T("s67") FS_BT_V                                                    \
+        "s_branch .Lfn_loop_%=\n"                                                                                   \
+        FS_NDZ_LOOP(PF, CNT)                                                                                        \
+        FS_FDU_LOOP("fn", PF, "", FS_PK_PN, FS_NDZ_LOAD, FS_NDZ_TAIL)  \
         "v_max_f32_e64 v62, |%[dcx]|, |%[dcy]|\n\t"                                                                 \
         "s_mov_b32 %[st], 0\n\t"                                                                                    \
         "v_ldexp_f32 v62, v62, 26\n\t"                                                                              \
@@ -242,12 +276,14 @@
         "s_waitcnt lgkmcnt(0)"                                                                                      \
         : "+{v[48:49]}"(wv), "={v[50:51]}"(r1), "={v[52:53]}"(r2), "={v[54:55]}"(r3), "={v[56:57]}"(ts_),           \
           "={v[58:59]}"(ta_), "+{v60}"(mxS), "={v61}"(tn_), "={v62}"(tl_), [t] "=&s"(bt_t_), [st] "=&s"(st),        \
-          "+{s67}"(pwi), "+{s[64:65]}"(zS), [off] "+s"(off), [pf] "=&s"(pf_), [pg] "=&s"(pg_), [ph] "=&s"(ph_)      \
+          "+{s67}"(pwi), "+{s[64:65]}"(zS), [off] "+s"(off), [pf] "=&s"(pf_), [pg] "=&s"(pg_), [ph] "=&s"(ph_),     \
+          [nz] "+s"(nz_)                                                                                            \
         : [se] "v"(sE2), [dc] "v"(dcs), [dcx] "v"(dcs.x), [dcy] "v"(dcs.y), [eshm] "s"(Esh_cap),                    \
-          [sdc] "s"(sdc_bits), [lim8] "s"(lim8), [nd] "s"(nd_sel), "{s[68:69]}"(zpb), [flr] "s"(kFloorBits)         \
+          [sdc] "s"(sdc_bits), [lim8] "s"(lim8), [nd] "s"(nd_sel), "{s[68:69]}"(zpb), "{s[70:71]}"(znp),            \
+          [flr] "s"(kFloorBits)                                                                                     \
         : "s36", "s37", "s38", "s39", "s40", "s41", "s42", "s43", "s44", "s45", "s46", "s47", "s48", "s49", "s50",  \
-          "s51", "s52", "s53", "s54", "s55", "s56", "s57", "s58", "s59", "s60", "s61", "s62", "s63", "s66", "vcc",  \
-          "scc")
+          "s51", "s52", "s53", "s54", "s55", "s56", "s57", "s58", "s59", "s60", "s61", "s62", "s63", "s66", "s72",  \
+          "vcc", "scc")
 constexpr uint32_t kNdBackoffEntry = 8;
 constexpr uint32_t kNdBackoffVerdict = 32;
 
diff --git a/include/fsmi355_internal.h b/include/fsmi355_internal.h
--- a/include/fsmi355_internal.h
+++ b/include/fsmi355_internal.h
@@ -30,6 +30,8 @@
 uint32_t fs_read_stats_raw(fs_renderer *r, uint64_t *out, uint64_t max_words);
 uint32_t fs_test_block_threshold(fs_renderer *r, const int32_t *bound_bits, const int32_t *scale_shift, const int32_t *dc_bits,
                                  int32_t *threshold_out, uint32_t n);
+uint32_t fs_test_ndz_threshold(fs_renderer *r, const int32_t *bound_bits, const int32_t *scale_shift, const int32_t *dc_bits,
+                               int32_t *threshold_out, uint32_t n);
 uint32_t fs_time_render_current(fs_renderer *r, uint64_t n_iterations, uint32_t repeats, float ms_out[2]);
 
 
```

Measured after the change: 223.3 Mpix/s, median of 6. +6.1%, better.
